# alpc91/SGRL

Measured on AMD Instinct MI355X. Metric: env-steps/sec (whole node) + SET-actor fwd us/step, 3d_walker mix @8192 envs/GPU, higher is better.
Workload: dtype f64 (dynamics) / f32 (SET actor, obs); 1 GPU; 3D_Walker++ 8 variants x 1024 envs per GPU (config 3), random U(-1,1) actions, auto-reset, SET actor forward on every step, random-init weights; envs_per_gpu=8192, obs_max_len=287, action_max_len=21, replay_gather=none (single rank)

## Files before the change

### include/sgrl_set.h

```cpp
#ifndef SGRL_SET_H
#define SGRL_SET_H

#include <stdint.h>

#ifdef __cplusplus
extern "C" {
#endif

typedef struct sgrl_set sgrl_set;

enum {
  SGRL_SET_EMB0 = 0, SGRL_SET_EMB1, SGRL_SET_EMB2, SGRL_SET_REL_W, SGRL_SET_REL_B, SGRL_SET_FNORM_W, SGRL_SET_FNORM_B,
  SGRL_SET_GENC, SGRL_SET_ENC_W, SGRL_SET_ENC_B, SGRL_SET_GGPROJ, SGRL_SET_L1G_W, SGRL_SET_L1G_B, SGRL_SET_L2G_W,
  SGRL_SET_L2G_B, SGRL_SET_L1NG_W, SGRL_SET_L1NG_B, SGRL_SET_L2NG_W, SGRL_SET_L2NG_B, SGRL_SET_DECG, SGRL_SET_L1M_W,
  SGRL_SET_L1M_B, SGRL_SET_L2M_W, SGRL_SET_L2M_B, SGRL_SET_GPROJ,
  SGRL_SET_NGLOBAL
};
enum {
  SGRL_SET_A_GPROJ = 0, SGRL_SET_A_LG1_W, SGRL_SET_A_LG1_B, SGRL_SET_A_LG2_W, SGRL_SET_A_LG2_B, SGRL_SET_QKV_W,
  SGRL_SET_QKV_B, SGRL_SET_VG_W, SGRL_SET_NGOUT_W, SGRL_SET_NGOUT_B, SGRL_SET_GOUT_W, SGRL_SET_F_GPROJ2,
  SGRL_SET_F_GPROJ3, SGRL_SET_F_LG1_W, SGRL_SET_F_LG1_B, SGRL_SET_F_LG2_W, SGRL_SET_F_LG2_B, SGRL_SET_L3_W,
  SGRL_SET_L3_B, SGRL_SET_L4_W, SGRL_SET_L4_B, SGRL_SET_L5_W, SGRL_SET_L1_W, SGRL_SET_L1_B, SGRL_SET_L2_W,
  SGRL_SET_L2_B, SGRL_SET_N1_W, SGRL_SET_N1_B, SGRL_SET_N2_W, SGRL_SET_N2_B, SGRL_SET_A_GD,
  SGRL_SET_NLAYER
};
#define SGRL_SET_LAYERS 3
#define SGRL_SET_NW (SGRL_SET_NGLOBAL + SGRL_SET_LAYERS * SGRL_SET_NLAYER)

int sgrl_set_create(sgrl_set** out);
void sgrl_set_destroy(sgrl_set* s);

int sgrl_set_weights(sgrl_set* s, const float* w, const int64_t* offsets, int n_offsets);

enum { SGRL_PACK_COPY = 0, SGRL_PACK_PADCOL = 1, SGRL_PACK_FOLD = 2, SGRL_PACK_STACK = 3, SGRL_PACK_MATMUL = 4, SGRL_PACK_SUBMAT = 5,
       SGRL_PACK_PERM32 = 6 };
typedef struct sgrl_pack_seg {
  int64_t dst;
  const void* src0;
  const void* src1;
  int32_t n;
  int32_t kind;
  int32_t a, b;
  float scale;
  int32_t lda, ldb;
  int32_t reserved;
} sgrl_pack_seg;
#define SGRL_SET_NSITES 7
#define SGRL_SET_NEXTRA 2
int sgrl_set_bind_params(sgrl_set* s, const sgrl_pack_seg* segs, int n_segs, const int64_t* offsets, int n_offsets,
                         int64_t total_floats);

int sgrl_set_hold_weights(sgrl_set* s, int hold);

int sgrl_set_graph(sgrl_set* s, int n_morph, const int32_t* morph_L, const int32_t* morph_count, const int32_t* trav,
                   const float* rel);
#define SGRL_SET_GRAPH_CACHE 128

int sgrl_set_forward(sgrl_set* s, const float* obs, int obs_ld, float* act, int act_ld, float max_action, void* stream);

int sgrl_set_forward_q(sgrl_set* s, const float* obs, int obs_ld, const float* action, int action_ld, float* q, int q_ld,
                       void* stream);

int sgrl_set_num_nodes(const sgrl_set* s);
int64_t sgrl_set_workspace_bytes(const sgrl_set* s);
int64_t sgrl_set_generation(const sgrl_set* s);
int sgrl_set_time_forward(sgrl_set* s, const float* obs, int obs_ld, float* act, int act_ld, float max_action,
                          int reps, void* stream, float* ms_out);
int sgrl_set_peek(sgrl_set* s, int which, float* host, int64_t n_floats);
int sgrl_set_debug_stop_after(sgrl_set* s, int stage);
int sgrl_set_debug_small_nodes(sgrl_set* s, int nodes);
int sgrl_set_last_split(const sgrl_set* s);
#define SGRL_SET_FORM_F16X3 2
#define SGRL_SET_FORM_BF16X6 3
int sgrl_set_gemm_form(sgrl_set* s, int form);
int sgrl_set_debug_product(sgrl_set* s, int kind, int form, const float* A, int lda, const float* W, int ldw, const float* bias,
                           float* C, int ldc, int M, int N, int K, const float* rowdiv, const float* aux_in, float* aux_out,
                           void* stream);
int sgrl_set_debug_chain(sgrl_set* s, int kind, const float* A, int lda, int K, const float* Wp, const float* W1, const float* b1, int hid,
                         const float* W2, const float* b2, float* C, int ldc, int M, const float* rowdiv, const float* ln, float* zc,
                         float* z2, float* fn, void* stream);
long long sgrl_set_debug_redos(int reset);
const char* sgrl_set_last_error(void);

#ifdef __cplusplus
}
#endif
#endif
```

### sgrl_amd/csrc/set_actor.hip

```cpp
#include <hip/hip_runtime.h>

#include <algorithm>
#include <cmath>
#include <cstdint>
#include <cstdlib>
#include <cstring>
#include <string>
#include <type_traits>
#include <vector>

#include "../../include/sgrl.h"
#include "../../include/sgrl_set.h"
#include "../../include/sgrl_train.h"
#include "gemm_f32.h"
#include "chain_f16.h"
#include "stream_pick.h"

namespace {

thread_local std::string g_set_err;
int sfail(int code, const std::string& msg) { g_set_err = msg; return code; }
#define SHIP_TRY(expr)                                                                     \
  do {                                                                                     \
    hipError_t _e = (expr);                                                                \
    if (_e != hipSuccess) return sfail(SGRL_ERR_HIP, std::string(#expr) + ": " + hipGetErrorString(_e)); \
  } while (0)

constexpr int D = 128;
constexpr int ZD = 32;
constexpr int GK = sgrl_gemm::kGramK;
constexpr int OGLD = 144;

using sgrl_gemm::EPI_ACC2;
using sgrl_gemm::EPI_EQUIV;
using sgrl_gemm::EPI_LN;
using sgrl_gemm::EPI_RELU;
using sgrl_gemm::EPI_ROWDIV;
using sgrl_gemm::EPI_ZSPLIT;
using sgrl_gemm::GemmArgs;
using sgrl_gemm::k_gemm2;

__device__ __forceinline__ float wave_sum_f32(float v) {
  for (int off = 32; off > 0; off >>= 1) v += __shfl_xor(v, off, 64);
  return v;
}

struct NodeTab {
  const int32_t* node_env;
  const int32_t* node_limb;
  const int32_t* node_mnode;
  const int32_t* trav;
  int TM;
};
constexpr int kEmbedNodes = 8;
__global__ __launch_bounds__(128) void k_embed(const float* __restrict__ obs, int obs_ld, const float* __restrict__ action,
                                               int act_ld, int ngf, NodeTab nt, const float* Wge, const float* We,
                                               const float* be, const float* e0, const float* e1, const float* e2, float* g,
                                               float* cat, float* outg, float* outng, float* gdir, float* zc, float* z2, int N) {
  __shared__ float os[kEmbedNodes][44];
  const int n0 = blockIdx.x * kEmbedNodes, c = threadIdx.x;
  for (int idx = c; idx < kEmbedNodes * 44; idx += 128) {
    const int q = idx / 44, k = idx % 44, n = n0 + q;
    float v = 0.f;
    if (n < N) {
      const int env = nt.node_env[n], limb = nt.node_limb[n];
      if (k < 41) v = obs[(size_t)env * obs_ld + 41 * limb + k];
      else if (action) v = action[(size_t)env * act_ld + 3 * limb + (k - 41)];
    }
    os[q][k] = v;
  }
  float wg[8], we[20];
#pragma unroll
  for (int j = 0; j < 8; j++) wg[j] = Wge[c * 8 + j];
#pragma unroll
  for (int j = 0; j < 20; j++) we[j] = j < ngf ? We[c * ngf + j] : 0.f;
  const float bias = be[c];
  __syncthreads();
  const float sc = sqrtf(128.f);
  for (int q = 0; q < kEmbedNodes; q++) {
    const int n = n0 + q;
    if (n >= N) break;
    const float* o = os[q];
    const int mn = nt.node_mnode[n];
    for (int s = 0; s < 3; s++) {
      float v = 0.f;
#pragma unroll
      for (int j = 0; j < 8; j++) v += wg[j] * o[3 * j + s];
      g[((size_t)n * 3 + s) * D + c] = v * sc;
    }
    float v = bias;
#pragma unroll
    for (int j = 0; j < 20; j++) if (j < ngf) v += we[j] * o[24 + j];
    float pos;
    if (c < 42) pos = e0[nt.trav[mn] * 42 + c];
    else if (c < 84) pos = e1[nt.trav[nt.TM + mn] * 42 + (c - 42)];
    else pos = e2[nt.trav[2 * nt.TM + mn] * 44 + (c - 84)];
    cat[(size_t)n * 256 + 128 + c] = v * sc + pos;
    if (c < 24) { const int s = c / 8, j = c % 8; outg[((size_t)n * 3 + s) * OGLD + j] = o[3 * j + s]; }
    if (c < ngf) outng[(size_t)n * 160 + c] = o[24 + c];
    if (c >= ngf && c < 32) outng[(size_t)n * 160 + 128 + c] = 0.f;
    if (c < 6) {
      const int s = c / 2, e = c % 2;
      const float gv = o[3 * (1 + e) + s];
      gdir[((size_t)n * 3 + s) * 2 + e] = gv;
      zc[((size_t)n * 3 + s) * ZD + 30 + e] = gv;
      z2[((size_t)n * 3 + s) * ZD + 30 + e] = gv;
    }
  }
}

__global__ void k_stack_proj(const float* __restrict__ Wp, const float* __restrict__ Wq, int C, int Cpad, float* out) {
  for (int i = blockIdx.x * blockDim.x + threadIdx.x; i < 64 * Cpad; i += gridDim.x * blockDim.x) {
    const int r = i / Cpad, c = i % Cpad;
    float v = 0.f;
    if (c < C) {
      if (r < 30) v = Wp[r * C + c];
      else if (Wq && r >= 32 && r < 62) v = Wq[(r - 32) * C + c];
    }
    out[i] = v;
  }
}

constexpr int PACK_CHUNK = 4096;
constexpr int PACK_CHUNK_MM = 256;
__global__ __launch_bounds__(256) void k_pack(const sgrl_pack_seg* __restrict__ segs, const int2* __restrict__ chunks,
                                              const unsigned short* __restrict__ tri, float* w) {
  const int2 ch = chunks[blockIdx.x];
  const sgrl_pack_seg sg = segs[ch.x];
  const float* s0 = static_cast<const float*>(sg.src0);
  const float* s1 = static_cast<const float*>(sg.src1);
  const int end = min(ch.y + (sg.kind == SGRL_PACK_MATMUL ? PACK_CHUNK_MM : PACK_CHUNK), sg.n);
  for (int i = ch.y + (int)threadIdx.x; i < end; i += 256) {
    float v = 0.f;
    switch (sg.kind) {
      case SGRL_PACK_COPY:
        if (i < sg.a) v = s0[i] * sg.scale;
        break;
      case SGRL_PACK_PADCOL: {
        const int r = i / sg.b, c = i % sg.b;
        if (c < sg.a) v = s0[(size_t)r * sg.a + c];
        break;
      }
      case SGRL_PACK_FOLD: {
        const int r = i / GK, k = i % GK;
        const unsigned short t = tri[k];
        if (t != 0xFFFF) {
          const int aa = t >> 8, bb = t & 255;
          const float* row = s0 + (size_t)r * (ZD * ZD);
          v = (aa == bb) ? row[aa * ZD + bb] : row[aa * ZD + bb] + row[bb * ZD + aa];
        }
        break;
      }
      case SGRL_PACK_STACK: {
        const int r = i / sg.b, c = i % sg.b;
        if (c < sg.a) {
          if (r < 30) v = s0[r * sg.a + c];
          else if (s1 && r >= 32 && r < 62) v = s1[(r - 32) * sg.a + c];
        }
        break;
      }
      case SGRL_PACK_MATMUL: {
        const int r = i / sg.b, c = i % sg.b;
        const float* ar = s0 + (size_t)r * sg.lda;
        float acc = 0.f;
        int k = 0;
        for (; k + 8 <= sg.a; k += 8) {
          float x[8], y[8];
#pragma unroll
          for (int u = 0; u < 8; u++) { x[u] = ar[k + u]; y[u] = s1[(size_t)(k + u) * sg.ldb + c]; }
#pragma unroll
          for (int u = 0; u < 8; u++) acc += x[u] * y[u];
        }
        for (; k < sg.a; k++) acc += ar[k] * s1[(size_t)k * sg.ldb + c];
        v = acc * sg.scale;
        break;
      }
      case SGRL_PACK_PERM32: {
        const int r = i / sg.a, k = i % sg.a;
        v = s0[(size_t)((r & 31) * 32 + (r >> 5)) * sg.a + k];
        break;
      }
      case SGRL_PACK_SUBMAT: {
        const int r = i / sg.b, c = i % sg.b;
        v = s0[(size_t)r * sg.lda + c];
        break;
      }
      default: break;
    }
    w[sg.dst + i] = v;
  }
}

__global__ void k_relbias(const float* rel, const float* Wr, const float* br, float* relb, const int32_t* m_off,
                          const int32_t* m_L, int n_morph) {
  const int k = blockIdx.x;
  if (k >= n_morph) return;
  const int L = m_L[k], off = m_off[k];
  for (int i = threadIdx.x; i < 2 * L * L; i += blockDim.x) {
    const int h = i / (L * L), ij = i % (L * L);
    const float* r = rel + (size_t)(off / 2) * 3 + ij * 3;
    relb[off + i] = Wr[h * 3] * r[0] + Wr[h * 3 + 1] * r[1] + Wr[h * 3 + 2] * r[2] + br[h];
  }
}

struct EnvTab {
  const int32_t* env_off;
  const int32_t* env_L;
  const int32_t* env_relb;
};
__global__ __launch_bounds__(256) void k_attention(const float* __restrict__ qkv, const float* __restrict__ U,
                                                   const float* __restrict__ gdir, const float* relb, EnvTab et,
                                                   int use_bias, const float* __restrict__ b_ng, const float* __restrict__ GD,
                                                   float* delta_dbg, float* g1, float* ng, int ng_ld,
                                                   const float* __restrict__ ln_w, const float* __restrict__ ln_b) {
  constexpr int LMAX = 14;
  __shared__ float sc[2 * LMAX * LMAX];
  __shared__ float gd[2 * LMAX * 3 * 2];
  __shared__ float dl[LMAX][128];
  const int e = blockIdx.x, t = threadIdx.x;
  const int n0 = et.env_off[e], L = et.env_L[e];
  {
    const int sub = t & 7;
    for (int idx = t >> 3; idx < 2 * L * L; idx += 32) {
      const int h = idx / (L * L), i = (idx / L) % L, j = idx % L;
      const float4* q = reinterpret_cast<const float4*>(qkv + (size_t)(n0 + i) * 768 + h * 128);
      const float4* k = reinterpret_cast<const float4*>(qkv + (size_t)(n0 + j) * 768 + 256 + h * 128);
      float s = 0.f;
#pragma unroll
      for (int u = 0; u < 4; u++) {
        const float4 a = q[sub + 8 * u], b = k[sub + 8 * u];
        s += a.x * b.x + a.y * b.y + a.z * b.z + a.w * b.w;
      }
      s += __shfl_xor(s, 1, 64); s += __shfl_xor(s, 2, 64); s += __shfl_xor(s, 4, 64);
      if (sub == 0) sc[idx] = use_bias ? s + relb[et.env_relb[e] + idx] : s;
    }
  }
  __syncthreads();
  if (t < 2 * L) {
    float* row = sc + t * L;
    float mx = row[0];
    for (int j = 1; j < L; j++) mx = fmaxf(mx, row[j]);
    float sum = 0.f;
    for (int j = 0; j < L; j++) { row[j] = expf(row[j] - mx); sum += row[j]; }
    for (int j = 0; j < L; j++) row[j] = row[j] / sum;
  }
  __syncthreads();
  for (int idx = t; idx < 2 * L * 6; idx += 256) {
    const int h = idx / (L * 6), i = (idx / 6) % L, se = idx % 6;
    const float* w = sc + (h * L + i) * L;
    float s = 0.f;
    for (int j = 0; j < L; j++) s += w[j] * gdir[(size_t)(n0 + j) * 6 + se];
    gd[idx] = s;
  }
  __syncthreads();
  {
    const int quantity = t >> 6, ln = t & 63, h = ln >> 5, c4 = (ln & 31) * 4;
    const float* vbase = quantity == 0 ? qkv + (size_t)n0 * 768 + 512 + h * 128 + c4
                                       : U + ((size_t)n0 * 3 + (quantity - 1)) * 256 + h * 128 + c4;
    auto body = [&](auto ltc, const int i0) __attribute__((always_inline)) {
      constexpr int LT = decltype(ltc)::value;
      float4 out[LT];
#pragma unroll
      for (int i = 0; i < LT; i++) out[i] = make_float4(0.f, 0.f, 0.f, 0.f);
      const float* wh = sc + h * L * L;
      if (L <= 8) {
#pragma unroll
        for (int jb = 0; jb < 8; jb += 4) {
          if (jb >= L) break;
          float4 v[4];
#pragma unroll
          for (int j = 0; j < 4; j++)
            v[j] = jb + j < L ? *reinterpret_cast<const float4*>(vbase + (size_t)(jb + j) * 768) : make_float4(0.f, 0.f, 0.f, 0.f);
#pragma unroll
          for (int j = 0; j < 4; j++)
            if (jb + j < L) {
#pragma unroll
              for (int i = 0; i < LT; i++)
                if (i0 + i < L) {
                  const float w = wh[(i0 + i) * L + jb + j];
                  out[i].x += w * v[j].x; out[i].y += w * v[j].y; out[i].z += w * v[j].z; out[i].w += w * v[j].w;
                }
            }
        }
      } else {
        float4 v = *reinterpret_cast<const float4*>(vbase);
        for (int j = 0; j < L; j++) {
          const float4 vn = *reinterpret_cast<const float4*>(vbase + (size_t)(j + 1 < L ? j + 1 : j) * 768);
#pragma unroll
          for (int i = 0; i < LT; i++)
            if (i0 + i < L) {
              const float w = wh[(i0 + i) * L + j];
              out[i].x += w * v.x; out[i].y += w * v.y; out[i].z += w * v.z; out[i].w += w * v.w;
            }
          v = vn;
        }
      }
      if (quantity != 0) {
        const float4 ga = *reinterpret_cast<const float4*>(GD + (h * 128 + c4) * 2);
        const float4 gb = *reinterpret_cast<const float4*>(GD + (h * 128 + c4) * 2 + 4);
#pragma unroll
        for (int i = 0; i < LT; i++)
          if (i0 + i < L) {
            const float* gg = gd + (h * L + i0 + i) * 6 + 2 * (quantity - 1);
            const float g0 = gg[0], g1v = gg[1];
            out[i].x += ga.x * g0 + ga.y * g1v; out[i].y += ga.z * g0 + ga.w * g1v;
            out[i].z += gb.x * g0 + gb.y * g1v; out[i].w += gb.z * g0 + gb.w * g1v;
          }
      }
      float4 bb = make_float4(0.f, 0.f, 0.f, 0.f);
      if (quantity == 0) bb = *reinterpret_cast<const float4*>(b_ng + c4);
#pragma unroll
      for (int i = 0; i < LT; i++)
        if (i0 + i < L) {
          float4 o = out[i];
          const float px = __shfl_xor(o.x, 32, 64), py = __shfl_xor(o.y, 32, 64), pz = __shfl_xor(o.z, 32, 64), pw = __shfl_xor(o.w, 32, 64);
          o = h == 0 ? make_float4(o.x + px, o.y + py, o.z + pz, o.w + pw) : make_float4(px + o.x, py + o.y, pz + o.z, pw + o.w);
          if ((i & 1) == h) {
            if (quantity != 0) {
              *reinterpret_cast<float4*>(g1 + ((size_t)(n0 + i0 + i) * 3 + (quantity - 1)) * 128 + c4) = o;
            } else {
              o.x += bb.x; o.y += bb.y; o.z += bb.z; o.w += bb.w;
              *reinterpret_cast<float4*>(&dl[i0 + i][c4]) = o;
              if (delta_dbg) *reinterpret_cast<float4*>(delta_dbg + (size_t)(n0 + i0 + i) * 128 + c4) = o;
            }
          }
        }
    };
    for (int i0 = 0; i0 < L; i0 += 4) body(std::integral_constant<int, 4>{}, i0);
  }
  __syncthreads();
  const int lane = t & 63;
  const float w0 = ln_w[lane], w1 = ln_w[64 + lane], b0 = ln_b[lane], b1 = ln_b[64 + lane];
  for (int i = t >> 6; i < L; i += 4) {
    float* row = ng + (size_t)(n0 + i) * ng_ld;
    const float v0 = row[lane] + dl[i][lane], v1 = row[64 + lane] + dl[i][64 + lane];
    const float mu = wave_sum_f32(v0 + v1) * (1.f / 128.f);
    const float d0 = v0 - mu, d1 = v1 - mu;
    const float var = wave_sum_f32(d0 * d0 + d1 * d1) * (1.f / 128.f);
    const float inv = 1.0f / sqrtf(var + 1e-5f);
    row[lane] = d0 * inv * w0 + b0;
    row[64 + lane] = d1 * inv * w1 + b1;
  }
}

__global__ __launch_bounds__(256) void k_add_ln(const float* x, int ldx, const float* delta, int ldd, const float* w,
                                                const float* b, float* out1, int ld1, float* out2, int ld2, int N) {
  const int row = blockIdx.x * 4 + (threadIdx.x >> 6), lane = threadIdx.x & 63;
  if (row >= N) return;
  float v0 = x[(size_t)row * ldx + lane], v1 = x[(size_t)row * ldx + 64 + lane];
  if (delta) { v0 += delta[(size_t)row * ldd + lane]; v1 += delta[(size_t)row * ldd + 64 + lane]; }
  const float mu = wave_sum_f32(v0 + v1) * (1.f / 128.f);
  const float d0 = v0 - mu, d1 = v1 - mu;
  const float var = wave_sum_f32(d0 * d0 + d1 * d1) * (1.f / 128.f);
  const float inv = 1.0f / sqrtf(var + 1e-5f);
  const float y0 = d0 * inv * w[lane] + b[lane], y1 = d1 * inv * w[64 + lane] + b[64 + lane];
  if (out1) { out1[(size_t)row * ld1 + lane] = y0; out1[(size_t)row * ld1 + 64 + lane] = y1; }
  if (out2) { out2[(size_t)row * ld2 + lane] = y0; out2[(size_t)row * ld2 + 64 + lane] = y1; }
}

__global__ __launch_bounds__(128) void k_equiv(const float* __restrict__ T, const float* __restrict__ W5,
                                               const float* __restrict__ g1, float* g, float* outg, int N) {
  __shared__ float Ts[8 * 96];
  const int t = threadIdx.x, n0 = blockIdx.x * 8;
  const int rows = min(8, N - n0) * 3;
  for (int o = t; o < 8 * 96; o += 128) Ts[o] = (n0 + o / 96 < N) ? T[(size_t)n0 * 96 + o] : 0.f;
  float w[32];
#pragma unroll
  for (int c = 0; c < 32; c++) w[c] = W5[t * 32 + c];
  __syncthreads();
#pragma unroll
  for (int rb = 0; rb < 24; rb += 8) {
    if (rb >= rows) break;
    float gv[8], g1v[8];
#pragma unroll
    for (int r = 0; r < 8; r++) {
      const size_t row = (size_t)n0 * 3 + (rb + r < rows ? rb + r : 0);
      gv[r] = g[row * D + t];
      g1v[r] = g1[row * D + t];
    }
#pragma unroll
    for (int r = 0; r < 8; r++) {
      if (rb + r >= rows) break;
      const float* tt = Ts + (rb + r) * 32;
      float v = 0.f;
#pragma unroll
      for (int c = 0; c < 32; c++) v += tt[c] * w[c];
      const size_t row = (size_t)n0 * 3 + rb + r;
      const float gn = gv[r] + (g1v[r] + v);
      g[row * D + t] = gn;
      if (outg) {
        outg[row * OGLD + 8 + t] = gn;
        if (t < OGLD - 136) outg[row * OGLD + 136 + t] = 0.f;
      }
    }
  }
}

__global__ __launch_bounds__(128) void k_head_out(const float* __restrict__ T, const float* __restrict__ wdec,
                                                  const float* __restrict__ obs, int obs_ld, NodeTab nt, float* act, int act_ld,
                                                  float max_action, int N) {
  const int n = blockIdx.x * 4 + (threadIdx.x >> 5), c = threadIdx.x & 31;
  if (n >= N) return;
  float vec[3];
  const float wd = wdec[c];
  for (int s = 0; s < 3; s++) {
    float v = T[(size_t)n * 96 + s * 32 + c] * wd;
    for (int off = 16; off > 0; off >>= 1) v += __shfl_xor(v, off, 32);
    vec[s] = v;
  }
  if (c < 3) {
    const int env = nt.node_env[n], limb = nt.node_limb[n];
    const float* o = obs + (size_t)env * obs_ld + 41 * limb + 3 * (5 + c);
    const float a = o[0] * vec[0] + o[1] * vec[1] + o[2] * vec[2];
    act[(size_t)env * act_ld + 3 * limb + c] = max_action * tanhf(a);
  }
}


__global__ __launch_bounds__(128) void k_head_out2(const float* __restrict__ m2, const float* __restrict__ z, const float* __restrict__ obs,
                                                   int obs_ld, NodeTab nt, float* act, int act_ld, float max_action, int N) {
  const int n = blockIdx.x * 4 + (threadIdx.x >> 5), c = threadIdx.x & 31;
  if (n >= N) return;
  float vec[3];
  const float mq = m2[(size_t)n * 32 + c];
  for (int s = 0; s < 3; s++) {
    float v = z[(size_t)n * 96 + s * 32 + c] * mq;
    for (int off = 16; off > 0; off >>= 1) v += __shfl_xor(v, off, 32);
    vec[s] = v;
  }
  if (c < 3) {
    const int env = nt.node_env[n], limb = nt.node_limb[n];
    const float* o = obs + (size_t)env * obs_ld + 41 * limb + 3 * (5 + c);
    const float a = o[0] * vec[0] + o[1] * vec[1] + o[2] * vec[2];
    act[(size_t)env * act_ld + 3 * limb + c] = max_action * tanhf(a);
  }
}

__global__ __launch_bounds__(256) void k_q_head(const float* __restrict__ c, const float* __restrict__ w, const float* __restrict__ b,
                                                const float* __restrict__ fn, NodeTab nt, float* q, int q_ld, int N) {
  const int n = blockIdx.x * 4 + (threadIdx.x >> 6), lane = threadIdx.x & 63;
  if (n >= N) return;
  const float* row = c + (size_t)n * 256;
  float v = row[lane] * w[lane] + row[64 + lane] * w[64 + lane] + row[128 + lane] * w[128 + lane] + row[192 + lane] * w[192 + lane];
  v = wave_sum_f32(v);
  if (lane == 0) q[(size_t)nt.node_env[n] * q_ld + nt.node_limb[n]] = (v + b[0]) / fn[n];
}

}

struct GraphCfg {
  std::vector<int32_t> key_i;
  std::vector<float> key_f;
  int n_env = 0, N = 0, n_morph = 0, TM = 0, Lmax = 0;
  int split_env = 0, split_node = 0;
  int32_t *d_node_env = nullptr, *d_node_limb = nullptr, *d_node_mnode = nullptr, *d_trav = nullptr;
  int32_t *d_env_off = nullptr, *d_env_L = nullptr, *d_env_relb = nullptr, *d_m_off = nullptr, *d_m_L = nullptr;
  float *d_rel = nullptr, *d_relb = nullptr;
  uint64_t last_use = 0;
  void release() {
    void* ptrs[] = {d_node_env, d_node_limb, d_node_mnode, d_trav, d_env_off, d_env_L, d_env_relb, d_m_off, d_m_L, d_rel, d_relb};
    for (void* q : ptrs) if (q) (void)hipFree(q);
  }
};

struct sgrl_set {
  const float* w = nullptr;
  int64_t off[SGRL_SET_NW];
  bool have_w = false, have_graph = false;
  int n_env = 0, N = 0, n_morph = 0, TM = 0, Lmax = 0;
  int split_env = 0, split_node = 0;
  int last_split = 0;
  int32_t *d_node_env = nullptr, *d_node_limb = nullptr, *d_node_mnode = nullptr, *d_trav = nullptr;
  int32_t *d_env_off = nullptr, *d_env_L = nullptr, *d_env_relb = nullptr, *d_m_off = nullptr, *d_m_L = nullptr;
  float *d_rel = nullptr, *d_relb = nullptr;
  std::vector<GraphCfg*> cfgs;
  uint64_t use_clock = 0;
  int64_t generation = 0;
  float* ws = nullptr;
  int64_t ws_floats = 0;
  int carved_N = 0;
  float* cat_cur = nullptr;
  float *g, *cat, *cat2, *zc, *fn, *h256, *qkv, *vg, *g1, *z2, *mat, *t256, *t256b, *t128a, *t128b, *delta,
      *outg, *outng, *gdir;
  float* wstack = nullptr;
  const float* site_ptr[SGRL_SET_NSITES];
  bool hold = false, packed_ok = false;
  int packed_form = 0;
  hipEvent_t ev_pack = nullptr;
  const float* l2mf_w = nullptr;
  const float* l2mf_b = nullptr;
  unsigned short* d_tri = nullptr;
  bool stack_dirty = true;
  bool stack_critic = false;
  int stop_after = -1;
  int small_nodes = -1;
  int gemm_form = 0;
  sgrl_gemm::EncMat* d_enc = nullptr;
  int n_enc = 0, enc_rows = 0;
  float* wsc = nullptr;
  std::vector<std::pair<int64_t, int>> enc_index;
  bool live = false;
  float* wflat = nullptr;
  unsigned* wwords = nullptr;
  int64_t wflat_floats = 0;
  sgrl_pack_seg* d_segs = nullptr;
  int2* d_chunks = nullptr;
  int n_chunks = 0;
  hipStream_t side = nullptr;
  hipEvent_t ev_fork = nullptr, ev_join = nullptr, ev_l3 = nullptr;
  hipEvent_t ev_fork_b = nullptr, ev_join_b = nullptr, ev_split = nullptr, ev_merge = nullptr;
  std::vector<hipStream_t> side_ok_for;
  int side_picks = 0;
  const float* W(int slot) const { return w + off[slot]; }
  const float* WL(int layer, int k) const { return w + off[SGRL_SET_NGLOBAL + layer * SGRL_SET_NLAYER + k]; }
};

namespace {

constexpr int64_t kPerNodeFloats = 384  + 256 + 256  + 96  + 1  + 256  + 768  +
                                   768  + 384  + 96  + 96  + 256 + 256  +
                                   128 + 128 + 128  + 3 * OGLD  + 160  + 6 ;
constexpr int kWsArrays = 19;

int64_t ws_floats_for(int64_t N) { return kPerNodeFloats * N + 32 * kWsArrays; }

void free_graphs(sgrl_set* s) {
  for (GraphCfg* c : s->cfgs) { c->release(); delete c; }
  s->cfgs.clear();
  if (s->ws) (void)hipFree(s->ws);
  s->ws = nullptr; s->ws_floats = 0; s->carved_N = 0;
  s->have_graph = false;
}

template <class T>
int upload(T** dst, const std::vector<T>& v) {
  if (hipMalloc(dst, sizeof(T) * (v.size() ? v.size() : 1)) != hipSuccess) return -1;
  if (!v.empty() && hipMemcpy(*dst, v.data(), sizeof(T) * v.size(), hipMemcpyHostToDevice) != hipSuccess) return -1;
  return 0;
}

void pick_split(const std::vector<int32_t>& env_off, int N, int* env_out, int* node_out) {
  int best = 0, best_rank = -1;
  int64_t best_dist = 0;
  for (size_t e = 1; e < env_off.size(); e++) {
    const int n = env_off[e];
    const int64_t dist = std::abs(2 * (int64_t)n - N);
    const int rank = 2 * dist > N / 16 ? 0 : (n % 128 == 0 ? 3 : n % 64 == 0 ? 2 : 1);
    if (best_rank < 0 || rank > best_rank || (rank == best_rank && dist < best_dist)) { best = (int)e; best_rank = rank; best_dist = dist; }
  }
  *env_out = best;
  *node_out = best ? env_off[best] : 0;
}

int use_cfg(sgrl_set* s, GraphCfg* c) {
  const int64_t N = c->N;
  const int64_t need = ws_floats_for(N);
  if (need > s->ws_floats) {
    if (s->ws) { (void)hipFree(s->ws); s->generation++; }
    s->ws = nullptr; s->ws_floats = 0; s->carved_N = 0;
    if (hipMalloc(&s->ws, sizeof(float) * need) != hipSuccess) return sfail(SGRL_ERR_HIP, "device allocation failed (SET workspace)");
    s->ws_floats = need;
  }
  if (s->carved_N != c->N) {
    float* p = s->ws;
    auto take = [&](int64_t n) { float* r = p; p += (n + 31) & ~int64_t(31); return r; };
    s->g = take(384 * N); s->cat = take(256 * N); s->cat2 = take(256 * N); s->zc = take(96 * N); s->fn = take(N);
    s->h256 = take(256 * N); s->qkv = take(768 * N); s->vg = take(768 * N);
    s->g1 = take(384 * N); s->z2 = take(96 * N); s->mat = take(96 * N); s->t256 = take(256 * N); s->t256b = take(256 * N); s->t128a = take(128 * N);
    s->t128b = take(128 * N); s->delta = take(128 * N); s->outg = take(3 * OGLD * N); s->outng = take(160 * N); s->gdir = take(6 * N);
    if (p - s->ws > s->ws_floats) return sfail(SGRL_ERR_LIMIT, "workspace carve-up overflow");
    s->carved_N = c->N;
  }
  s->n_env = c->n_env; s->N = c->N; s->n_morph = c->n_morph; s->TM = c->TM; s->Lmax = c->Lmax;
  s->split_env = c->split_env; s->split_node = c->split_node;
  s->d_node_env = c->d_node_env; s->d_node_limb = c->d_node_limb; s->d_node_mnode = c->d_node_mnode; s->d_trav = c->d_trav;
  s->d_env_off = c->d_env_off; s->d_env_L = c->d_env_L; s->d_env_relb = c->d_env_relb; s->d_m_off = c->d_m_off; s->d_m_L = c->d_m_L;
  s->d_rel = c->d_rel; s->d_relb = c->d_relb;
  c->last_use = ++s->use_clock;
  s->have_graph = true;
  return SGRL_OK;
}

bool gemm_use_split() {
  static const bool v = [] { const char* e = getenv("SGRL_SET_GEMM"); return !(e && e[0] == 'f'); }();
  return v;
}
struct GemmCtx {
  int form = SGRL_SET_FORM_F16X3;
  const float* w_base = nullptr; const unsigned* w_words = nullptr;
  const float* wsc = nullptr;
  const std::vector<std::pair<int64_t, int>>* enc_index = nullptr;
};
int gemm_default_form() {
  static const int v = [] { const char* e = getenv("SGRL_SET_GEMM"); return (e && e[0] == 'b') ? SGRL_SET_FORM_BF16X6 : SGRL_SET_FORM_F16X3; }();
  return v;
}
const float* wsc_of(const GemmCtx& gx, const float* W) {
  if (!gx.enc_index) return nullptr;
  const int64_t off = W - gx.w_base;
  for (const auto& e : *gx.enc_index) if (e.first == off) return gx.wsc + e.second;
  return nullptr;
}
GemmArgs with_words(const GemmCtx& gx, const GemmArgs& a) {
  GemmArgs b = a;
  b.W = reinterpret_cast<const float*>(gx.w_words + (a.W - gx.w_base));
  b.wscale = wsc_of(gx, a.W);
  return b;
}
template <int F> struct GemmKernels {
  static constexpr auto kNarrow = k_gemm2<F, 4, 1, 1, 2, 16, 1>;
  static constexpr auto kWide = k_gemm2<F, 4, 2, 1, 2, 32, 2>;
  static constexpr auto kSquare = k_gemm2<F, 4, 4, 1, 1, 32, 2>;
  static constexpr auto kSplit = sgrl_gemm::k_gemm3<F, 4, 2, 1, 2, 16, 2>;
  static constexpr auto kSplitH = sgrl_gemm::k_gemm3<F, 4, 2, 1, 2, 16, 2, false, false, false, 0, false, 2, true, 2>;
  static constexpr int kSplitHLds = sgrl_gemm::TileCfg3<4, 2, 1, 2, 16, 2>::kLdsBytes;
  static constexpr int kNarrowLds = sgrl_gemm::TileCfg<4, 1, 1, 2, 16>::kLdsBytes;
  static constexpr int kWideLds = sgrl_gemm::TileCfg<4, 2, 1, 2, 32>::kLdsBytes;
  static constexpr int kSquareLds = sgrl_gemm::TileCfg<4, 4, 1, 1, 32>::kLdsBytes;
  static constexpr int kSplitLds = sgrl_gemm::TileCfg3<4, 2, 1, 2, 16>::kLdsBytes;
  static bool raise_lds_limits() {
    return hipFuncSetAttribute(reinterpret_cast<const void*>(kNarrow), hipFuncAttributeMaxDynamicSharedMemorySize, kNarrowLds) == hipSuccess &&
           hipFuncSetAttribute(reinterpret_cast<const void*>(kWide), hipFuncAttributeMaxDynamicSharedMemorySize, kWideLds) == hipSuccess &&
           hipFuncSetAttribute(reinterpret_cast<const void*>(kSquare), hipFuncAttributeMaxDynamicSharedMemorySize, kSquareLds) == hipSuccess &&
           hipFuncSetAttribute(reinterpret_cast<const void*>(kSplit), hipFuncAttributeMaxDynamicSharedMemorySize, kSplitLds) == hipSuccess &&
           hipFuncSetAttribute(reinterpret_cast<const void*>(kSplitH), hipFuncAttributeMaxDynamicSharedMemorySize, kSplitHLds) == hipSuccess;
  }
  static void launch(const GemmCtx& gx, hipStream_t st, const GemmArgs& a) {
    const int tiles128 = ((a.M + 127) / 128) * ((a.N + 127) / 128);
    if (a.N <= 64 || (a.K % 32) != 0) {
      hipLaunchKernelGGL(kNarrow, dim3(((a.M + 127) / 128) * ((a.N + 63) / 64)), dim3(256), kNarrowLds, st, a);
    } else if (gemm_use_split()) {
      if (gx.form == SGRL_SET_FORM_F16X3) hipLaunchKernelGGL(kSplitH, dim3(tiles128), dim3(512), kSplitHLds, st, with_words(gx, a));
      else hipLaunchKernelGGL(kSplit, dim3(tiles128), dim3(512), kSplitLds, st, a);
    } else if (tiles128 < 512) {
      hipLaunchKernelGGL(kNarrow, dim3(((a.M + 127) / 128) * ((a.N + 63) / 64)), dim3(256), kNarrowLds, st, a);
    } else if (a.N >= 512) {
      hipLaunchKernelGGL(kWide, dim3(tiles128), dim3(512), kWideLds, st, a);
    } else {
      hipLaunchKernelGGL(kSquare, dim3(tiles128), dim3(1024), kSquareLds, st, a);
    }
  }
};

constexpr auto kProjH = sgrl_gemm::k_gemm3<EPI_ZSPLIT, 4, 1, 1, 2, 16, 2, false, false, false, 0, false, 2, false, 2>;
constexpr int kProjHLds = sgrl_gemm::TileCfg3<4, 1, 1, 2, 16, 2>::kLdsBytes;

constexpr auto kGemmEquiv = sgrl_gemm::k_gemm3<EPI_ROWDIV | EPI_EQUIV, 4, 2, 1, 2, 16, 2>;
constexpr auto kGemmEquivH = sgrl_gemm::k_gemm3<EPI_ROWDIV | EPI_EQUIV, 4, 2, 1, 2, 16, 2, false, false, false, 0, false, 2, true, 2>;
constexpr int kEquivLds = GemmKernels<0>::kSplitLds > 128 * 100 * 4 ? GemmKernels<0>::kSplitLds : 128 * 100 * 4;
int launch_gemm_equiv(const GemmCtx& gx, hipStream_t st, const float* A, int lda, const float* W, int ldw, const float* bias, int M, int K,
                      const float* rowdiv, const float* zq, float* tout) {
  if (K % 32 != 0 || (lda & 3) || (ldw & 3)) return sfail(SGRL_ERR_ARG, "gemm_equiv: K must be a multiple of 32 and rows 16-byte aligned");
  GemmArgs a{A, lda, W, ldw, bias, nullptr, 0, M, 1024, K, EPI_ROWDIV | EPI_EQUIV, rowdiv, nullptr, 0};
  a.zq = zq; a.tout = tout;
  if (gx.form == SGRL_SET_FORM_F16X3) hipLaunchKernelGGL(kGemmEquivH, dim3(((M + 127) / 128) * 8), dim3(512), kEquivLds, st, with_words(gx, a));
  else hipLaunchKernelGGL(kGemmEquiv, dim3(((M + 127) / 128) * 8), dim3(512), kEquivLds, st, a);
  return SGRL_OK;
}

constexpr auto kGemmGram = sgrl_gemm::k_gemm3<EPI_RELU, 4, 2, 1, 2, 16, 2, false, false, false, 0, true>;
constexpr auto kGemmGramH = sgrl_gemm::k_gemm3<EPI_RELU, 4, 2, 1, 2, 16, 2, false, false, false, 0, true, 2, true, 2>;
int launch_gemm_gram(const GemmCtx& gx, hipStream_t st, const float* zc, const float* W, const float* bias, float* C, int ldc, int M, int N, float* fn) {
  if (N % 128 != 0) return sfail(SGRL_ERR_ARG, "gemm_gram: N must be a multiple of 128");
  GemmArgs a{zc, 96, W, GK, bias, C, ldc, M, N, GK, EPI_RELU, nullptr, nullptr, 0};
  a.rowdiv_out = fn;
  if (gx.form == SGRL_SET_FORM_F16X3) hipLaunchKernelGGL(kGemmGramH, dim3(((M + 127) / 128) * (N / 128)), dim3(512), GemmKernels<0>::kSplitHLds, st, with_words(gx, a));
  else hipLaunchKernelGGL(kGemmGram, dim3(((M + 127) / 128) * (N / 128)), dim3(512), GemmKernels<0>::kSplitLds, st, a);
  return SGRL_OK;
}

constexpr auto kGemmLn = sgrl_gemm::k_gemm3<EPI_ROWDIV | EPI_LN, 4, 2, 1, 2, 16, 2>;
constexpr auto kGemmLnH = sgrl_gemm::k_gemm3<EPI_ROWDIV | EPI_LN, 4, 2, 1, 2, 16, 2, false, false, false, 0, false, 2, true, 2>;
int launch_gemm_ln(const GemmCtx& gx, hipStream_t st, const float* A, int lda, const float* W, int ldw, const float* bias, int M, int K,
                   const float* rowdiv, float* ln_io, int ln_ld, const float* ln_w, const float* ln_b) {
  if (K % 32 != 0 || (lda & 3) || (ldw & 3)) return sfail(SGRL_ERR_ARG, "gemm_ln: K must be a multiple of 32 and rows 16-byte aligned");
  GemmArgs a{A, lda, W, ldw, bias, nullptr, 0, M, 128, K, EPI_ROWDIV | EPI_LN, rowdiv, nullptr, 0};
  a.ln_io = ln_io; a.ln_ld = ln_ld; a.ln_w = ln_w; a.ln_b = ln_b;
  if (gx.form == SGRL_SET_FORM_F16X3) hipLaunchKernelGGL(kGemmLnH, dim3((M + 127) / 128), dim3(512), GemmKernels<0>::kSplitHLds, st, with_words(gx, a));
  else hipLaunchKernelGGL(kGemmLn, dim3((M + 127) / 128), dim3(512), GemmKernels<0>::kSplitLds, st, a);
  return SGRL_OK;
}

int launch_gemm(const GemmCtx& gx, hipStream_t st, const float* A, int lda, const float* W, int ldw, const float* bias, float* C, int ldc,
                int M, int N, int K, int flags = 0, const float* rowdiv = nullptr, float* C2 = nullptr, int ldc2 = 0) {
  if (K % 16 != 0 || (lda & 3) || (ldw & 3)) return sfail(SGRL_ERR_ARG, "gemm: K must be a multiple of 16 and rows 16-byte aligned");
  GemmArgs a{A, lda, W, ldw, bias, C, ldc, M, N, K, flags, rowdiv, C2, ldc2};
  switch (flags) {
    case 0: GemmKernels<0>::launch(gx, st, a); break;
    case EPI_RELU: GemmKernels<EPI_RELU>::launch(gx, st, a); break;
    case EPI_ROWDIV: GemmKernels<EPI_ROWDIV>::launch(gx, st, a); break;
    case EPI_ACC2: GemmKernels<EPI_ACC2>::launch(gx, st, a); break;
    default: return sfail(SGRL_ERR_ARG, "gemm: unsupported epilogue combination");
  }
  return SGRL_OK;
}

bool chain_enabled() {
  static const bool v = [] { const char* e = getenv("SGRL_SET_CHAIN"); return !(e && e[0] == '0'); }();
  return v;
}
using sgrl_gemm::ChainArgs;
using sgrl_gemm::k_chain;
constexpr auto kSiteA = k_chain<1, 256, 0, 1>;
constexpr auto kSiteF = k_chain<1, 256, 0, 2>;
constexpr auto kSiteH1 = k_chain<1, 128, 0, 1>;
constexpr auto kSiteH2 = k_chain<1, 128, 0, 2>;
constexpr auto kChainLn = k_chain<0, 256, EPI_ROWDIV | EPI_LN, 0>;
constexpr auto kChainNg = k_chain<0, 128, 0, 0>;
constexpr auto kChainPlain = k_chain<0, 256, 0, 0>;
bool chain_raise_lds_limits() {
  const void* ks[] = {reinterpret_cast<const void*>(kSiteA), reinterpret_cast<const void*>(kSiteF), reinterpret_cast<const void*>(kSiteH1),
                      reinterpret_cast<const void*>(kSiteH2), reinterpret_cast<const void*>(kChainLn), reinterpret_cast<const void*>(kChainNg),
                      reinterpret_cast<const void*>(kChainPlain)};
  for (const void* k : ks)
    if (hipFuncSetAttribute(k, hipFuncAttributeMaxDynamicSharedMemorySize, sgrl_gemm::kChainLds) != hipSuccess) return false;
  return hipFuncSetAttribute(reinterpret_cast<const void*>(k_chain<0, 256, EPI_ROWDIV | EPI_EQUIV, 0>), hipFuncAttributeMaxDynamicSharedMemorySize,
                             sgrl_gemm::kChainEqLds) == hipSuccess;
}
const unsigned* words_of(const GemmCtx& gx, const float* W) { return gx.w_words + (W - gx.w_base); }
int launch_site(const GemmCtx& gx, hipStream_t st, const float* X, int ldx, int Kp, const float* Wp, float* zc, float* z2, float* fn, const float* W1,
                const float* b1, int hid, const float* W2, const float* b2, float* C, int ldc, int M) {
  if (Kp % 16 != 0 || (ldx & 3) || (hid != 256 && hid != 128)) return sfail(SGRL_ERR_ARG, "site: K must be a multiple of 16, rows 16-byte aligned, hidden width 128 or 256");
  ChainArgs a{};
  a.A = zc; a.W1 = words_of(gx, W1); a.ldw1 = GK; a.b1 = b1; a.W2 = words_of(gx, W2); a.ldw2 = hid; a.b2 = b2; a.C = C; a.ldc = ldc; a.M = M; a.K1 = GK;
  a.fn_out = fn; a.X = X; a.ldx = ldx; a.Kp = Kp; a.Wp = words_of(gx, Wp); a.zc = zc; a.z2 = z2;
  a.ws1 = wsc_of(gx, W1); a.ws2 = wsc_of(gx, W2); a.wsp = wsc_of(gx, Wp);
  if (!a.ws1 || !a.ws2 || !a.wsp) return sfail(SGRL_ERR_ARG, "site: a weight operand is not a matrix of the row-scale table");
  const dim3 grid((M + sgrl_gemm::kChainRows - 1) / sgrl_gemm::kChainRows);
  if (hid == 256) {
    if (z2) hipLaunchKernelGGL(kSiteF, grid, dim3(512), sgrl_gemm::kChainLds, st, a);
    else hipLaunchKernelGGL(kSiteA, grid, dim3(512), sgrl_gemm::kChainLds, st, a);
  } else {
    if (z2) hipLaunchKernelGGL(kSiteH2, grid, dim3(512), sgrl_gemm::kChainLds, st, a);
    else hipLaunchKernelGGL(kSiteH1, grid, dim3(512), sgrl_gemm::kChainLds, st, a);
  }
  return SGRL_OK;
}
int launch_chain_ln(const GemmCtx& gx, hipStream_t st, const float* A, int lda, int K1, const float* W1, const float* b1, const float* W2, const float* b2,
                    const float* rowdiv, float* ln_io, int ln_ld, const float* ln_w, const float* ln_b, int M, float* ln_out = nullptr) {
  if (K1 % 16 != 0 || (lda & 3)) return sfail(SGRL_ERR_ARG, "chain: K must be a multiple of 16 and rows 16-byte aligned");
  ChainArgs a{};
  a.A = A; a.lda = lda; a.W1 = words_of(gx, W1); a.ldw1 = K1; a.b1 = b1; a.W2 = words_of(gx, W2); a.ldw2 = 256; a.b2 = b2; a.M = M; a.K1 = K1;
  a.rowdiv = rowdiv; a.ln_io = ln_io; a.ln_ld = ln_ld; a.ln_w = ln_w; a.ln_b = ln_b; a.ln_out = ln_out;
  a.ws1 = wsc_of(gx, W1); a.ws2 = wsc_of(gx, W2);
  if (!a.ws1 || !a.ws2) return sfail(SGRL_ERR_ARG, "chain: a weight operand is not a matrix of the row-scale table");
  hipLaunchKernelGGL(kChainLn, dim3((M + sgrl_gemm::kChainRows - 1) / sgrl_gemm::kChainRows), dim3(512), sgrl_gemm::kChainLds, st, a);
  return SGRL_OK;
}
constexpr auto kChainEq = k_chain<0, 256, EPI_ROWDIV | EPI_EQUIV, 0>;
int launch_chain_ng(const GemmCtx& gx, hipStream_t st, const float* A, int lda, int K1, const float* W1, const float* b1, const float* W2, const float* b2,
                    float* C, int ldc, int M) {
  if (K1 % 16 != 0 || (lda & 3)) return sfail(SGRL_ERR_ARG, "chain: K must be a multiple of 16 and rows 16-byte aligned");
  ChainArgs a{};
  a.A = A; a.lda = lda; a.W1 = words_of(gx, W1); a.ldw1 = K1; a.b1 = b1; a.W2 = words_of(gx, W2); a.ldw2 = 128; a.b2 = b2; a.C = C; a.ldc = ldc; a.M = M;
  a.K1 = K1; a.ws1 = wsc_of(gx, W1); a.ws2 = wsc_of(gx, W2);
  if (!a.ws1 || !a.ws2) return sfail(SGRL_ERR_ARG, "chain: a weight operand is not a matrix of the row-scale table");
  hipLaunchKernelGGL(kChainNg, dim3((M + sgrl_gemm::kChainRows - 1) / sgrl_gemm::kChainRows), dim3(512), sgrl_gemm::kChainLds, st, a);
  return SGRL_OK;
}

constexpr int kSmallNodesDefault = 2048;
constexpr int kSplitMinNodes = 2048;

__global__ __launch_bounds__(256) void k_gram576(const float* __restrict__ zc, const unsigned short* __restrict__ tri,
                                                 float* __restrict__ A, float* __restrict__ fn, int N) {
  __shared__ float zs[4][96];
  const int w = threadIdx.x >> 6, lane = threadIdx.x & 63, node = blockIdx.x * 4 + w;
  const bool live = node < N;
  if (live) {
    zs[w][lane] = zc[(size_t)node * 96 + lane];
    if (lane < 32) zs[w][64 + lane] = zc[(size_t)node * 96 + 64 + lane];
  }
  __syncthreads();
  if (!live) return;
  float ss = 0.f;
  for (int k = lane; k < GK; k += 64) {
    const unsigned t = tri[k];
    float v = 0.f;
    if (t != 0xFFFFu) {
      const int a = t >> 8, b = t & 255;
      v = zs[w][a] * zs[w][b] + zs[w][32 + a] * zs[w][32 + b] + zs[w][64 + a] * zs[w][64 + b];
      ss += (a == b ? 1.f : 2.f) * v * v;
    }
    A[(size_t)node * GK + k] = v;
  }
  ss = wave_sum_f32(ss);
  if (lane == 0) fn[node] = sqrtf(ss) + 1.f;
}

__global__ __launch_bounds__(128) void k_zmat_perm(const float* __restrict__ zq, const float* __restrict__ matp,
                                                   float* __restrict__ tout) {
  __shared__ float ms[32 * 33], zs[96];
  const int t = threadIdx.x;
  const size_t n = blockIdx.x;
  for (int o = t; o < 1024; o += 128) ms[(o >> 5) * 33 + (o & 31)] = matp[n * 1024 + o];
  if (t < 96) zs[t] = zq[n * 96 + t];
  __syncthreads();
  if (t >= 96) return;
  const int sI = t >> 5, c = t & 31;
  float acc = 0.f;
#pragma unroll
  for (int a = 0; a < 32; a++) acc += zs[sI * 32 + a] * ms[c * 33 + a];
  tout[n * 96 + t] = acc;
}

int small_fail() { return sfail(SGRL_ERR_HIP, std::string("small-batch product: ") + sgrl_train_last_error()); }

int small_gemm(hipStream_t st, const float* A, int lda, const float* W, int ldw, const float* bias, float* C, int ldc, int M,
               int N, int K, int flags = 0, const float* rowdiv = nullptr) {
  if (flags & ~(EPI_RELU | EPI_ROWDIV)) return sfail(SGRL_ERR_ARG, "small gemm: unsupported epilogue");
  const int rc = sgrl_linear_forward(A, lda, W, ldw, bias, (flags & EPI_ROWDIV) ? rowdiv : nullptr, C, ldc, M, N, K,
                                     (flags & EPI_RELU) ? 1 : 0, st);
  return rc == SGRL_OK ? rc : small_fail();
}

struct Part {
  int r0, M, e0, ne;
  hipStream_t st, sd;
  hipEvent_t ev_fork, ev_join;
  hipEvent_t ev_site0;
  float *catc, *cato, *g, *zc, *z2, *fn, *h256, *qkv, *vg, *g1, *mat, *t256, *t256b, *t128a, *t128b, *delta, *outg, *outng;
  NodeTab nt;
};

constexpr int kStages = 4 * SGRL_SET_LAYERS + 2, kStop = 1;

struct Forward {
  sgrl_set* s;
  const float* obs; int obs_ld; float* act; int act_ld; float max_action;
  bool critic; const float* action; int action_ld;
  hipStream_t st, sd;
  bool capturing, one_stream;
  bool small, chain;
  int ngf;
  GemmCtx gx;
  NodeTab nt;
  EnvTab et;

  void fork(const Part& p) const { if (!one_stream && p.sd != p.st) { (void)hipEventRecord(p.ev_fork, p.st); (void)hipStreamWaitEvent(p.sd, p.ev_fork, 0); } }
  void join(const Part& p) const { if (!one_stream && p.sd != p.st) { (void)hipEventRecord(p.ev_join, p.sd); (void)hipStreamWaitEvent(p.st, p.ev_join, 0); } }

  Part part(int r0, int M, int e0, int ne, hipStream_t pst, hipStream_t psd, hipEvent_t ev_fork, hipEvent_t ev_join, hipEvent_t ev_site0) const {
    const size_t r = (size_t)r0;
    Part p{r0, M, e0, ne, pst, psd, ev_fork, ev_join, ev_site0};
    p.catc = s->cat + 256 * r; p.cato = s->cat2 + 256 * r; p.g = s->g + 384 * r; p.zc = s->zc + 96 * r; p.z2 = s->z2 + 96 * r; p.fn = s->fn + r;
    p.h256 = s->h256 + 256 * r; p.qkv = s->qkv + 768 * r; p.vg = s->vg + 768 * r; p.g1 = s->g1 + 384 * r; p.mat = s->mat + 96 * r;
    p.t256 = s->t256 + 256 * r; p.t256b = s->t256b + 256 * r; p.t128a = s->t128a + 128 * r; p.t128b = s->t128b + 128 * r;
    p.delta = s->delta + 128 * r; p.outg = s->outg + 3 * OGLD * r; p.outng = s->outng + 160 * r;
    p.nt = NodeTab{nt.node_env + r, nt.node_limb + r, nt.node_mnode + r, nt.trav, nt.TM};
    return p;
  }
  const float* site_w(int site) const { return s->live ? s->site_ptr[site] : s->wstack + (size_t)site * 64 * 128; }

  int gemm(hipStream_t q, const float* A, int lda, const float* W, int ldw, const float* bias, float* C, int ldc, int M, int N, int K,
           int flags = 0, const float* rowdiv = nullptr) const {
    return small ? small_gemm(q, A, lda, W, ldw, bias, C, ldc, M, N, K, flags, rowdiv) : launch_gemm(gx, q, A, lda, W, ldw, bias, C, ldc, M, N, K, flags, rowdiv);
  }
  int gram_gemm(const Part& p, const float* W, const float* b, float* C, int ldc, int Nout) const {
    if (!small) return launch_gemm_gram(gx, p.st, p.zc, W, b, C, ldc, p.M, Nout, p.fn);
    hipLaunchKernelGGL(k_gram576, dim3((p.M + 3) / 4), dim3(256), 0, p.st, p.zc, s->d_tri, p.qkv, p.fn, p.M);
    return small_gemm(p.st, p.qkv, GK, W, GK, b, C, ldc, p.M, Nout, GK, EPI_RELU);
  }
  int equiv_gemm(const Part& p, const float* A, const float* W, const float* b) const {
    if (!small) return launch_gemm_equiv(gx, p.st, A, 256, W, 256, b, p.M, 256, p.fn, p.z2, p.mat);
    const int rc = small_gemm(p.st, A, 256, W, 256, b, p.qkv, 1024, p.M, 1024, 256, EPI_ROWDIV, p.fn);
    if (rc != SGRL_OK) return rc;
    hipLaunchKernelGGL(k_zmat_perm, dim3(p.M), dim3(128), 0, p.st, p.z2, p.qkv, p.mat);
    return SGRL_OK;
  }
  int project(const Part& p, const float* X, int ldx, int K, int site, float* z2) const {
    if (K % 16 != 0 || (ldx & 3)) return sfail(SGRL_ERR_ARG, "projection: K must be a multiple of 16 and rows 16-byte aligned");
    if (small) {
      int rc = small_gemm(p.st, X, ldx, site_w(site), K, nullptr, p.zc, ZD, 3 * p.M, 30, K);
      if (rc == SGRL_OK && z2) rc = small_gemm(p.st, X, ldx, site_w(site) + (size_t)32 * K, K, nullptr, z2, ZD, 3 * p.M, 30, K);
      return rc;
    }
    GemmArgs a{X, ldx, site_w(site), K, nullptr, p.zc, ZD, 3 * p.M, z2 ? 64 : 32, K, EPI_ZSPLIT, nullptr, z2, ZD};
    if (gx.form == SGRL_SET_FORM_F16X3 && gemm_use_split())
      hipLaunchKernelGGL(kProjH, dim3(((a.M + 127) / 128) * ((a.N + 63) / 64)), dim3(256), kProjHLds, p.st, with_words(gx, a));
    else
      GemmKernels<EPI_ZSPLIT>::launch(gx, p.st, a);
    return SGRL_OK;
  }
  int site(const Part& p, const float* X, int ldx, int K, int site, float* z2, const float* W1, const float* b1, int hid, float* hbuf,
           const float* W2, const float* b2, float* C) const {
    if (chain) return launch_site(gx, p.st, X, ldx, K, site_w(site), p.zc, z2, p.fn, W1, b1, hid, W2, b2, C, 256, p.M);
    int rc = project(p, X, ldx, K, site, z2);
    if (rc == SGRL_OK) rc = gram_gemm(p, W1, b1, hbuf, hid, hid);
    if (rc == SGRL_OK) rc = gemm(p.st, hbuf, hid, W2, hid, b2, C, 256, p.M, 128, hid);
    return rc;
  }

  void prologue(const Part& whole) {
    const int N = s->N;
    (void)hipMemsetAsync(act, 0, sizeof(float) * (size_t)s->n_env * act_ld, st);
    const bool want_words = !small && gx.form == SGRL_SET_FORM_F16X3 && gemm_use_split();
    const bool reuse = s->live && s->hold && s->packed_ok && (!want_words || s->packed_form == SGRL_SET_FORM_F16X3) && !capturing;
    if (reuse) (void)hipStreamWaitEvent(st, s->ev_pack, 0);
    if (s->live && !reuse)
      hipLaunchKernelGGL(k_pack, dim3(s->n_chunks), dim3(256), 0, st, s->d_segs, s->d_chunks, s->d_tri, s->wflat);
    const bool encode = s->live && !reuse && want_words;
    if (encode) {
      fork(whole);
      hipLaunchKernelGGL(sgrl_gemm::k_encode_rows, dim3((s->enc_rows + 3) / 4), dim3(256), 0, sd, s->wflat, s->wwords, s->wsc, s->d_enc, s->n_enc,
                         s->enc_rows);
    }
    hipLaunchKernelGGL(k_relbias, dim3(s->n_morph), dim3(256), 0, st, s->d_rel, s->W(SGRL_SET_REL_W), s->W(SGRL_SET_REL_B),
                       s->d_relb, s->d_m_off, s->d_m_L, s->n_morph);
    hipLaunchKernelGGL(k_embed, dim3((N + kEmbedNodes - 1) / kEmbedNodes), dim3(128), 0, st, obs, obs_ld, action, action_ld, ngf, nt,
                       s->W(SGRL_SET_GENC), s->W(SGRL_SET_ENC_W), s->W(SGRL_SET_ENC_B), s->W(SGRL_SET_EMB0), s->W(SGRL_SET_EMB1),
                       s->W(SGRL_SET_EMB2), s->g, s->cat, s->outg, s->outng, s->gdir, s->zc, s->z2, N);
    if (encode) join(whole);
    if (s->live && !reuse && !capturing) {
      s->packed_ok = s->hold;
      s->packed_form = want_words ? SGRL_SET_FORM_F16X3 : SGRL_SET_FORM_BF16X6;
      if (s->hold) (void)hipEventRecord(s->ev_pack, st);
    }
    s->cat_cur = s->cat;
    if (!s->live && (s->stack_dirty || s->stack_critic != critic)) {
      s->stack_critic = critic;
      auto sw = [&](int site) { return s->wstack + (size_t)site * 64 * 128; };
      for (int l = 0; l < SGRL_SET_LAYERS; l++) {
        hipLaunchKernelGGL(k_stack_proj, dim3(32), dim3(256), 0, st, s->WL(l, SGRL_SET_A_GPROJ), (const float*)nullptr, D, D, sw(2 * l));
        hipLaunchKernelGGL(k_stack_proj, dim3(32), dim3(256), 0, st, s->WL(l, SGRL_SET_F_GPROJ2), s->WL(l, SGRL_SET_F_GPROJ3), D, D, sw(2 * l + 1));
      }
      hipLaunchKernelGGL(k_stack_proj, dim3(36), dim3(256), 0, st, s->W(SGRL_SET_GGPROJ), critic ? (const float*)nullptr : s->W(SGRL_SET_GPROJ), 136, OGLD, sw(6));
      s->stack_dirty = false;
    }
  }
  int attn_site(const Part& p, int l) const {
    fork(p);
    int rc = gemm(p.sd, p.g, D, s->WL(l, SGRL_SET_VG_W), D, nullptr, p.vg, 256, 3 * p.M, 256, D);
    if (rc == SGRL_OK)
      rc = site(p, p.g, D, D, 2 * l, nullptr, s->WL(l, SGRL_SET_A_LG1_W), s->WL(l, SGRL_SET_A_LG1_B), 256, p.h256, s->WL(l, SGRL_SET_A_LG2_W),
                s->WL(l, SGRL_SET_A_LG2_B), p.catc);
    if (rc != SGRL_OK) return rc;
    if (l == 0 && p.ev_site0) (void)hipEventRecord(p.ev_site0, p.st);
    rc = gemm(p.st, p.catc, 256, s->WL(l, SGRL_SET_QKV_W), 256, s->WL(l, SGRL_SET_QKV_B), p.qkv, 768, p.M, 768, 256, EPI_ROWDIV, p.fn);
    if (rc != SGRL_OK) return rc;
    join(p);
    return SGRL_OK;
  }
  int attention(const Part& p, int l) const {
    const EnvTab etp{et.env_off + p.e0, et.env_L + p.e0, et.env_relb + p.e0};
    hipLaunchKernelGGL(k_attention, dim3(p.ne), dim3(256), 0, p.st, s->qkv, s->vg, s->gdir, s->d_relb, etp, l == 0 ? 1 : 0,
                       s->WL(l, SGRL_SET_NGOUT_B), s->WL(l, SGRL_SET_A_GD), s->stop_after == 2 * l ? s->delta : (float*)nullptr,
                       s->g1, p.catc - 256 * (size_t)p.r0 + 128, 256, s->WL(l, SGRL_SET_N1_W), s->WL(l, SGRL_SET_N1_B));
    return s->stop_after == 2 * l ? kStop : SGRL_OK;
  }
  int ffn_site(const Part& p, int l) const {
    return site(p, p.g1, D, D, 2 * l + 1, p.z2, s->WL(l, SGRL_SET_F_LG1_W), s->WL(l, SGRL_SET_F_LG1_B), 256, p.h256, s->WL(l, SGRL_SET_F_LG2_W),
                s->WL(l, SGRL_SET_F_LG2_B), p.catc);
  }
  int norm2_unfused(const Part& p, int l) const {
    float* const ng = p.catc + 128;
    if (!one_stream) {
      (void)hipEventRecord(s->ev_l3, p.st);
      (void)hipStreamWaitEvent(p.sd, s->ev_l3, 0);
    }
    if (!small)
      return launch_gemm_ln(gx, p.sd, p.t256b, 256, s->WL(l, SGRL_SET_L2_W), 256, s->WL(l, SGRL_SET_L2_B), p.M, 256, p.fn, ng, 256,
                            s->WL(l, SGRL_SET_N2_W), s->WL(l, SGRL_SET_N2_B));
    const int rc = small_gemm(p.st, p.t256b, 256, s->WL(l, SGRL_SET_L2_W), 256, s->WL(l, SGRL_SET_L2_B), p.delta, 128, p.M, 128, 256, EPI_ROWDIV, p.fn);
    if (rc != SGRL_OK) return rc;
    hipLaunchKernelGGL(k_add_ln, dim3((p.M + 3) / 4), dim3(256), 0, p.st, ng, 256, p.delta, 128, s->WL(l, SGRL_SET_N2_W),
                       s->WL(l, SGRL_SET_N2_B), (float*)nullptr, 0, ng, 256, p.M);
    return SGRL_OK;
  }
  int ffn_tail(Part& p, int l) const {
    fork(p);
    int rc;
    if (chain) {
      rc = launch_chain_ln(gx, p.sd, p.catc, 256, 256, s->WL(l, SGRL_SET_L1_W), s->WL(l, SGRL_SET_L1_B), s->WL(l, SGRL_SET_L2_W), s->WL(l, SGRL_SET_L2_B),
                           p.fn, p.catc + 128, 256, s->WL(l, SGRL_SET_N2_W), s->WL(l, SGRL_SET_N2_B), p.M, p.cato + 128);
    } else {
      rc = gemm(p.sd, p.catc, 256, s->WL(l, SGRL_SET_L1_W), 256, s->WL(l, SGRL_SET_L1_B), p.t256b, 256, p.M, 256, 256, EPI_RELU);
    }
    if (rc == SGRL_OK) rc = gemm(p.st, p.catc, 256, s->WL(l, SGRL_SET_L3_W), 256, s->WL(l, SGRL_SET_L3_B), p.t256, 256, p.M, 256, 256, EPI_RELU);
    if (rc == SGRL_OK && !chain) rc = norm2_unfused(p, l);
    if (rc == SGRL_OK) rc = equiv_gemm(p, p.t256, s->WL(l, SGRL_SET_L4_W), s->WL(l, SGRL_SET_L4_B));
    if (rc != SGRL_OK) return rc;
    hipLaunchKernelGGL(k_equiv, dim3((p.M + 7) / 8), dim3(128), 0, p.st, p.mat, s->WL(l, SGRL_SET_L5_W), p.g1, p.g,
                       l == SGRL_SET_LAYERS - 1 ? p.outg : (float*)nullptr, p.M);
    join(p);
    if (chain) {
      std::swap(p.catc, p.cato);
      s->cat_cur = p.catc - 256 * (size_t)p.r0;
    }
    return s->stop_after == 2 * l + 1 ? kStop : SGRL_OK;
  }
  int head_site(const Part& p) const {
    hipLaunchKernelGGL(k_add_ln, dim3((p.M + 3) / 4), dim3(256), 0, p.st, p.catc + 128, 256, (const float*)nullptr, 0, s->W(SGRL_SET_FNORM_W),
                       s->W(SGRL_SET_FNORM_B), (float*)nullptr, 0, p.outng + ngf, 160, p.M);
    fork(p);
    int rc;
    if (chain) {
      rc = launch_chain_ng(gx, p.sd, p.outng, 160, 160, s->W(SGRL_SET_L1NG_W), s->W(SGRL_SET_L1NG_B), s->W(SGRL_SET_L2NG_W), s->W(SGRL_SET_L2NG_B),
                           p.cato + 128, 256, p.M);
    } else {
      rc = gemm(p.sd, p.outng, 160, s->W(SGRL_SET_L1NG_W), 160, s->W(SGRL_SET_L1NG_B), p.t128b, D, p.M, D, 160, EPI_RELU);
      if (rc == SGRL_OK) rc = gemm(p.sd, p.t128b, D, s->W(SGRL_SET_L2NG_W), D, s->W(SGRL_SET_L2NG_B), p.cato + 128, 256, p.M, D, D);
    }
    if (rc == SGRL_OK)
      rc = site(p, p.outg, OGLD, OGLD, 6, critic ? (float*)nullptr : p.z2, s->W(SGRL_SET_L1G_W), s->W(SGRL_SET_L1G_B), 128, p.t128a,
                s->W(SGRL_SET_L2G_W), s->W(SGRL_SET_L2G_B), p.cato);
    if (rc != SGRL_OK) return rc;
    join(p);
    return SGRL_OK;
  }
  int head_out(const Part& p) const {
    const int N = p.M;
    if (critic) {
      hipLaunchKernelGGL(k_q_head, dim3((N + 3) / 4), dim3(256), 0, p.st, p.cato, s->W(SGRL_SET_DECG), s->W(SGRL_SET_L1M_B), p.fn, p.nt, act, act_ld, N);
      return SGRL_OK;
    }
    int rc = gemm(p.st, p.cato, 256, s->W(SGRL_SET_L1M_W), 256, s->W(SGRL_SET_L1M_B), p.t256, 256, N, 256, 256, EPI_RELU);
    if (rc != SGRL_OK) return rc;
    if (!small && s->live && s->l2mf_w) {
      rc = gemm(p.st, p.t256, 256, s->l2mf_w, 256, s->l2mf_b, p.mat, 32, N, 32, 256, EPI_ROWDIV, p.fn);
      if (rc != SGRL_OK) return rc;
      hipLaunchKernelGGL(k_head_out2, dim3((N + 3) / 4), dim3(128), 0, p.st, p.mat, p.z2, obs, obs_ld, p.nt, act, act_ld, max_action, N);
      return SGRL_OK;
    }
    rc = equiv_gemm(p, p.t256, s->W(SGRL_SET_L2M_W), s->W(SGRL_SET_L2M_B));
    if (rc != SGRL_OK) return rc;
    hipLaunchKernelGGL(k_head_out, dim3((N + 3) / 4), dim3(128), 0, p.st, p.mat, s->W(SGRL_SET_DECG), obs, obs_ld, p.nt, act, act_ld, max_action, N);
    return SGRL_OK;
  }
  int stage(Part& p, int k) const {
    const int l = k / 4;
    if (k == 4 * SGRL_SET_LAYERS) return head_site(p);
    if (k > 4 * SGRL_SET_LAYERS) return head_out(p);
    switch (k % 4) {
      case 0: return attn_site(p, l);
      case 1: return attention(p, l);
      case 2: return ffn_site(p, l);
      default: return ffn_tail(p, l);
    }
  }
};

GemmCtx gemm_ctx_of(const sgrl_set* s) {
  GemmCtx gx;
  gx.form = s->gemm_form ? s->gemm_form : gemm_default_form();
  if (!s->live || !s->wwords) gx.form = SGRL_SET_FORM_BF16X6;
  if (!gemm_use_split()) gx.form = SGRL_SET_FORM_BF16X6;
  gx.w_base = s->w; gx.w_words = s->wwords; gx.wsc = s->wsc; gx.enc_index = &s->enc_index;
  return gx;
}

int run_forward(sgrl_set* s, const float* obs, int obs_ld, float* act, int act_ld, float max_action, hipStream_t st,
                bool critic = false, const float* action = nullptr, int action_ld = 0) {
  const int N = s->N;
  Forward f{s, obs, obs_ld, act, act_ld, max_action, critic, action, action_ld, st};
  f.gx = gemm_ctx_of(s);
  f.ngf = critic ? 20 : 17;
  f.nt = NodeTab{s->d_node_env, s->d_node_limb, s->d_node_mnode, s->d_trav, s->TM};
  f.et = EnvTab{s->d_env_off, s->d_env_L, s->d_env_relb};
  f.small = N <= (s->small_nodes >= 0 ? s->small_nodes : kSmallNodesDefault);
  f.chain = !f.small && chain_enabled() && gemm_use_split() && f.gx.form == SGRL_SET_FORM_F16X3;
  hipStreamCaptureStatus cap = hipStreamCaptureStatusNone;
  (void)hipStreamIsCapturing(st, &cap);
  static const bool serial_env = [] { const char* e = getenv("SGRL_SET_ONE_STREAM"); return e && e[0] == '1'; }();
  f.capturing = cap != hipStreamCaptureStatusNone;
  f.one_stream = f.small || f.capturing || serial_env;
  if (!f.one_stream && sgrl_streams::enabled() && s->side_picks < 6 &&
      std::find(s->side_ok_for.begin(), s->side_ok_for.end(), st) == s->side_ok_for.end()) {
    s->side_picks++;
    hipStream_t chosen = sgrl_streams::pick({st}, s->side);
    if (chosen != s->side) s->side_ok_for.clear();
    s->side = chosen;
    s->side_ok_for.push_back(st);
  }
  hipStream_t sd = f.sd = f.one_stream ? st : s->side;
  Part whole = f.part(0, N, 0, s->n_env, st, sd, s->ev_fork, s->ev_join, nullptr);
  f.prologue(whole);
  static const int split_mode = [] { const char* e = getenv("SGRL_SET_SPLIT"); return e && e[0] >= '0' && e[0] <= '3' ? e[0] - '0' : 1; }();
  const bool split = split_mode != 0 && f.chain && !f.one_stream && s->stop_after < 0 && N >= kSplitMinNodes && s->split_node > 0 && s->split_node < N;
  s->last_split = split ? s->split_node : 0;
  if (!split) {
    for (int k = 0; k < kStages; k++) {
      const int rc = f.stage(whole, k);
      if (rc == kStop) return SGRL_OK;
      if (rc != SGRL_OK) return rc;
    }
  } else {
    const bool head_start = split_mode == 3;
    Part a = f.part(0, s->split_node, 0, s->split_env, st, sd, s->ev_fork, s->ev_join, head_start ? s->ev_split : (hipEvent_t) nullptr);
    Part b = f.part(s->split_node, N - s->split_node, s->split_env, s->n_env - s->split_env, sd, st, s->ev_fork_b, s->ev_join_b, nullptr);
    if (split_mode == 1) { a.sd = a.st; b.sd = b.st; }
    if (!head_start) (void)hipEventRecord(s->ev_split, st);
    for (int k = 0; k <= kStages; k++) {
      int rc = k < kStages ? f.stage(a, k) : SGRL_OK;
      if (rc != SGRL_OK) return rc;
      if (k == 0) (void)hipStreamWaitEvent(sd, s->ev_split, 0);
      if (k > 0) rc = f.stage(b, k - 1);
      if (rc != SGRL_OK) return rc;
    }
    (void)hipEventRecord(s->ev_merge, sd);
    (void)hipStreamWaitEvent(st, s->ev_merge, 0);
  }
  const hipError_t le = hipGetLastError();
  if (le != hipSuccess)
    return sfail(SGRL_ERR_HIP, std::string("kernel launch failed in sgrl_set_forward (") + hipGetErrorName(le) + ": " + hipGetErrorString(le) + ")");
  return SGRL_OK;
}

}

extern "C" {

int sgrl_set_create(sgrl_set** out) {
  if (!out) return sfail(SGRL_ERR_ARG, "out is null");
  int ndev = 0;
  if (hipGetDeviceCount(&ndev) != hipSuccess || ndev == 0) {
    *out = nullptr;
    return sfail(SGRL_ERR_HIP, "no HIP device visible: the SET actor fast path needs an MI355X (there is no CPU fallback)");
  }
  const bool attr_ok = hipFuncSetAttribute(reinterpret_cast<const void*>(kGemmEquiv), hipFuncAttributeMaxDynamicSharedMemorySize, kEquivLds) == hipSuccess &&
                       hipFuncSetAttribute(reinterpret_cast<const void*>(kGemmGram), hipFuncAttributeMaxDynamicSharedMemorySize, GemmKernels<0>::kSplitLds) == hipSuccess &&
                       hipFuncSetAttribute(reinterpret_cast<const void*>(kGemmLn), hipFuncAttributeMaxDynamicSharedMemorySize, GemmKernels<0>::kSplitLds) == hipSuccess &&
                       hipFuncSetAttribute(reinterpret_cast<const void*>(kGemmEquivH), hipFuncAttributeMaxDynamicSharedMemorySize, kEquivLds) == hipSuccess &&
                       hipFuncSetAttribute(reinterpret_cast<const void*>(kGemmGramH), hipFuncAttributeMaxDynamicSharedMemorySize, GemmKernels<0>::kSplitHLds) == hipSuccess &&
                       hipFuncSetAttribute(reinterpret_cast<const void*>(kGemmLnH), hipFuncAttributeMaxDynamicSharedMemorySize, GemmKernels<0>::kSplitHLds) == hipSuccess &&
                       GemmKernels<0>::raise_lds_limits() && GemmKernels<EPI_RELU>::raise_lds_limits() &&
                       GemmKernels<EPI_ROWDIV>::raise_lds_limits() && GemmKernels<EPI_ACC2>::raise_lds_limits() &&
                       GemmKernels<EPI_ZSPLIT>::raise_lds_limits() && chain_raise_lds_limits();
  if (!attr_ok) {
    *out = nullptr;
    return sfail(SGRL_ERR_HIP, "cannot raise the dynamic LDS limit of the GEMM kernel");
  }
  sgrl_set* s = new sgrl_set();
  std::vector<unsigned short> tri(GK, (unsigned short)0xFFFF);
  for (int A = 0, o = 0; A < ZD / 4; A++)
    for (int B = 0; B <= A; B++)
      for (int i = 0; i < 4; i++)
        for (int j = 0; j < 4; j++, o++)
          if (4 * A + i >= 4 * B + j) tri[o] = (unsigned short)(((4 * A + i) << 8) | (4 * B + j));
  const size_t wstack_floats = 6 * 64 * 128 + 64 * OGLD;
  if (hipStreamCreateWithFlags(&s->side, hipStreamNonBlocking) != hipSuccess ||
      hipEventCreateWithFlags(&s->ev_fork, hipEventDisableTiming) != hipSuccess ||
      hipEventCreateWithFlags(&s->ev_join, hipEventDisableTiming) != hipSuccess ||
      hipEventCreateWithFlags(&s->ev_l3, hipEventDisableTiming) != hipSuccess ||
      hipEventCreateWithFlags(&s->ev_fork_b, hipEventDisableTiming) != hipSuccess ||
      hipEventCreateWithFlags(&s->ev_join_b, hipEventDisableTiming) != hipSuccess ||
      hipEventCreateWithFlags(&s->ev_split, hipEventDisableTiming) != hipSuccess ||
      hipEventCreateWithFlags(&s->ev_merge, hipEventDisableTiming) != hipSuccess ||
      hipEventCreateWithFlags(&s->ev_pack, hipEventDisableTiming) != hipSuccess) {
    delete s;
    *out = nullptr;
    return sfail(SGRL_ERR_HIP, "cannot create the side stream of the SET actor");
  }
  if (hipMalloc(&s->wstack, sizeof(float) * wstack_floats) != hipSuccess || hipMalloc(&s->d_tri, sizeof(unsigned short) * GK) != hipSuccess ||
      hipMemcpy(s->d_tri, tri.data(), sizeof(unsigned short) * GK, hipMemcpyHostToDevice) != hipSuccess) {
    if (s->wstack) (void)hipFree(s->wstack);
    if (s->d_tri) (void)hipFree(s->d_tri);
    delete s;
    *out = nullptr;
    return sfail(SGRL_ERR_HIP, "device allocation failed in sgrl_set_create");
  }
  *out = s;
  return SGRL_OK;
}

void sgrl_set_destroy(sgrl_set* s) {
  if (!s) return;
  if (s->side) (void)hipStreamSynchronize(s->side);
  free_graphs(s);
  if (s->wstack) (void)hipFree(s->wstack);
  if (s->d_tri) (void)hipFree(s->d_tri);
  if (s->d_enc) (void)hipFree(s->d_enc);
  if (s->wsc) (void)hipFree(s->wsc);
  if (s->wflat) (void)hipFree(s->wflat);
  if (s->wwords) (void)hipFree(s->wwords);
  if (s->d_segs) (void)hipFree(s->d_segs);
  if (s->d_chunks) (void)hipFree(s->d_chunks);
  if (s->side) (void)hipStreamDestroy(s->side);
  if (s->ev_fork) (void)hipEventDestroy(s->ev_fork);
  if (s->ev_join) (void)hipEventDestroy(s->ev_join);
  if (s->ev_l3) (void)hipEventDestroy(s->ev_l3);
  for (hipEvent_t e : {s->ev_fork_b, s->ev_join_b, s->ev_split, s->ev_merge}) if (e) (void)hipEventDestroy(e);
  if (s->ev_pack) (void)hipEventDestroy(s->ev_pack);
  delete s;
}

int sgrl_set_weights(sgrl_set* s, const float* w, const int64_t* offsets, int n_offsets) {
  if (!s || !w || !offsets || n_offsets != SGRL_SET_NW) return sfail(SGRL_ERR_ARG, "sgrl_set_weights: bad argument");
  s->w = w;
  std::memcpy(s->off, offsets, sizeof(int64_t) * SGRL_SET_NW);
  s->have_w = true;
  s->live = false;
  s->l2mf_w = nullptr; s->l2mf_b = nullptr;
  s->stack_dirty = true;
  return SGRL_OK;
}

int sgrl_set_bind_params(sgrl_set* s, const sgrl_pack_seg* segs, int n_segs, const int64_t* offsets, int n_offsets,
                         int64_t total_floats) {
  if (!s || !segs || n_segs <= 0 || !offsets || n_offsets != SGRL_SET_NW + SGRL_SET_NSITES + SGRL_SET_NEXTRA || total_floats <= 0)
    return sfail(SGRL_ERR_ARG, "sgrl_set_bind_params: bad argument");
  std::vector<int> order(n_segs);
  for (int i = 0; i < n_segs; i++) order[i] = i;
  std::sort(order.begin(), order.end(), [&](int x, int y) { return segs[x].dst < segs[y].dst; });
  int64_t pos = 0;
  std::vector<int2> chunks;
  for (int oi = 0; oi < n_segs; oi++) {
    const sgrl_pack_seg& g = segs[order[oi]];
    if (g.dst != pos || g.n <= 0 || !g.src0) return sfail(SGRL_ERR_ARG, "sgrl_set_bind_params: segments must tile the buffer without gaps");
    bool ok = false;
    switch (g.kind) {
      case SGRL_PACK_COPY: ok = g.a >= 0 && g.a <= g.n; break;
      case SGRL_PACK_PADCOL: ok = g.a > 0 && g.b >= g.a && g.n % g.b == 0; break;
      case SGRL_PACK_FOLD: ok = g.n % GK == 0; break;
      case SGRL_PACK_STACK: ok = g.a > 0 && g.b >= g.a && g.n == 64 * g.b; break;
      case SGRL_PACK_MATMUL: ok = g.src1 && g.a > 0 && g.b > 0 && g.n % g.b == 0 && g.lda >= g.a && g.ldb >= g.b; break;
      case SGRL_PACK_SUBMAT: ok = g.b > 0 && g.n % g.b == 0 && g.lda >= g.b; break;
      case SGRL_PACK_PERM32: ok = g.a > 0 && g.n == 1024 * g.a; break;
      default: break;
    }
    if (!ok) return sfail(SGRL_ERR_ARG, "sgrl_set_bind_params: inconsistent segment " + std::to_string(order[oi]));
    for (int st = 0; st < g.n; st += (g.kind == SGRL_PACK_MATMUL ? PACK_CHUNK_MM : PACK_CHUNK)) chunks.push_back(make_int2(order[oi], st));
    pos += g.n;
  }
  if (pos != total_floats) return sfail(SGRL_ERR_ARG, "sgrl_set_bind_params: segments do not add up to total_floats");
  for (int k = 0; k < n_offsets; k++)
    if (offsets[k] < 0 || offsets[k] >= total_floats || (offsets[k] & 3)) return sfail(SGRL_ERR_ARG, "sgrl_set_bind_params: bad offset");
  if (s->wflat) s->generation++;
  if (s->wflat) (void)hipFree(s->wflat);
  if (s->wwords) (void)hipFree(s->wwords);
  if (s->d_segs) (void)hipFree(s->d_segs);
  if (s->d_chunks) (void)hipFree(s->d_chunks);
  s->wwords = nullptr;
  s->packed_ok = false;
  s->wflat = nullptr; s->d_segs = nullptr; s->d_chunks = nullptr; s->live = false; s->have_w = false;
  if (hipMalloc(&s->wflat, sizeof(float) * total_floats) != hipSuccess ||
      hipMalloc(&s->wwords, sizeof(unsigned) * total_floats) != hipSuccess ||
      hipMalloc(&s->d_segs, sizeof(sgrl_pack_seg) * n_segs) != hipSuccess ||
      hipMalloc(&s->d_chunks, sizeof(int2) * chunks.size()) != hipSuccess ||
      hipMemcpy(s->d_segs, segs, sizeof(sgrl_pack_seg) * n_segs, hipMemcpyHostToDevice) != hipSuccess ||
      hipMemcpy(s->d_chunks, chunks.data(), sizeof(int2) * chunks.size(), hipMemcpyHostToDevice) != hipSuccess)
    return sfail(SGRL_ERR_HIP, "device allocation failed in sgrl_set_bind_params");
  s->wflat_floats = total_floats;
  std::vector<int64_t> bounds(offsets, offsets + n_offsets);
  bounds.push_back(total_floats);
  std::sort(bounds.begin(), bounds.end());
  auto room = [&](int64_t off) { return *std::upper_bound(bounds.begin(), bounds.end(), off) - off; };
  {
    std::vector<sgrl_gemm::EncMat> mats;
    s->enc_index.clear();
    int rows_total = 0;
    auto add = [&](int64_t off, int rows, int K, int group = 1) {
      if (room(off) < (int64_t)rows * K) return;
      mats.push_back(sgrl_gemm::EncMat{off, rows, K, rows_total, group});
      s->enc_index.emplace_back(off, rows_total);
      rows_total += rows;
    };
    add(offsets[SGRL_SET_L1G_W], 128, GK); add(offsets[SGRL_SET_L2G_W], 128, 128);
    add(offsets[SGRL_SET_L1NG_W], 128, 160); add(offsets[SGRL_SET_L2NG_W], 128, 128);
    add(offsets[SGRL_SET_L1M_W], 256, 256); add(offsets[SGRL_SET_L2M_W], 1024, 256, 32);
    for (int l = 0; l < SGRL_SET_LAYERS; l++) {
      const int64_t* o = offsets + SGRL_SET_NGLOBAL + l * SGRL_SET_NLAYER;
      add(o[SGRL_SET_A_LG1_W], 256, GK); add(o[SGRL_SET_A_LG2_W], 128, 256); add(o[SGRL_SET_QKV_W], 768, 256); add(o[SGRL_SET_VG_W], 256, 128);
      add(o[SGRL_SET_F_LG1_W], 256, GK); add(o[SGRL_SET_F_LG2_W], 128, 256); add(o[SGRL_SET_L3_W], 256, 256); add(o[SGRL_SET_L4_W], 1024, 256, 32);
      add(o[SGRL_SET_L1_W], 256, 256); add(o[SGRL_SET_L2_W], 128, 256); add(o[SGRL_SET_L5_W], 128, 32);
    }
    for (int k = 0; k < SGRL_SET_NSITES; k++) add(offsets[SGRL_SET_NW + k], 64, k == 6 ? OGLD : 128);
    if (s->d_enc) (void)hipFree(s->d_enc);
    if (s->wsc) (void)hipFree(s->wsc);
    s->d_enc = nullptr; s->wsc = nullptr;
    s->n_enc = (int)mats.size(); s->enc_rows = rows_total;
    if (hipMalloc(&s->d_enc, sizeof(sgrl_gemm::EncMat) * mats.size()) != hipSuccess || hipMalloc(&s->wsc, sizeof(float) * rows_total) != hipSuccess ||
        hipMemcpy(s->d_enc, mats.data(), sizeof(sgrl_gemm::EncMat) * mats.size(), hipMemcpyHostToDevice) != hipSuccess)
      return sfail(SGRL_ERR_HIP, "device allocation failed in sgrl_set_bind_params (row-scale table)");
  }
  s->n_chunks = (int)chunks.size();
  s->w = s->wflat;
  std::memcpy(s->off, offsets, sizeof(int64_t) * SGRL_SET_NW);
  for (int k = 0; k < SGRL_SET_NSITES; k++) s->site_ptr[k] = s->wflat + offsets[SGRL_SET_NW + k];
  {
    const int64_t ow = offsets[SGRL_SET_NW + SGRL_SET_NSITES], ob = offsets[SGRL_SET_NW + SGRL_SET_NSITES + 1];
    const bool have = room(ow) >= 32 * 256;
    s->l2mf_w = have ? s->wflat + ow : nullptr;
    s->l2mf_b = have ? s->wflat + ob : nullptr;
  }
  s->live = true;
  s->have_w = true;
  return SGRL_OK;
}

int sgrl_set_graph(sgrl_set* s, int n_morph, const int32_t* morph_L, const int32_t* morph_count, const int32_t* trav,
                   const float* rel) {
  if (!s || n_morph <= 0 || !morph_L || !morph_count || !trav || !rel) return sfail(SGRL_ERR_ARG, "sgrl_set_graph: bad argument");
  std::vector<int32_t> key_i;
  size_t ntrav = 0, nrel = 0;
  for (int k = 0; k < n_morph; k++) {
    if (morph_L[k] < 2 || morph_L[k] > 14) return sfail(SGRL_ERR_LIMIT, "limb count must be in [2, 14]");
    if (morph_count[k] < 0) return sfail(SGRL_ERR_ARG, "negative morph_count");
    ntrav += 3 * (size_t)morph_L[k];
    nrel += 3 * (size_t)morph_L[k] * morph_L[k];
  }
  key_i.push_back(n_morph);
  key_i.insert(key_i.end(), morph_L, morph_L + n_morph);
  key_i.insert(key_i.end(), morph_count, morph_count + n_morph);
  key_i.insert(key_i.end(), trav, trav + ntrav);
  for (GraphCfg* c : s->cfgs)
    if (c->key_i == key_i && c->key_f.size() == nrel && std::memcmp(c->key_f.data(), rel, sizeof(float) * nrel) == 0)
      return use_cfg(s, c);
  std::vector<int32_t> node_env, node_limb, node_mnode, env_off, env_L, env_relb, m_off, m_L, travT;
  int TM = 0, relb_off = 0, env = 0, node = 0, Lmax = 0;
  std::vector<int> m_node0;
  for (int k = 0; k < n_morph; k++) {
    m_node0.push_back(TM);
    m_off.push_back(relb_off);
    m_L.push_back(morph_L[k]);
    TM += morph_L[k];
    relb_off += 2 * morph_L[k] * morph_L[k];
    if (morph_L[k] > Lmax) Lmax = morph_L[k];
  }
  travT.assign(3 * (size_t)TM, 0);
  {
    size_t tp = 0;
    for (int k = 0; k < n_morph; k++) {
      const int L = morph_L[k];
      for (int q = 0; q < 3; q++)
        for (int i = 0; i < L; i++) {
          const int v = trav[tp + q * L + i];
          if (v < 0 || v >= 15) return sfail(SGRL_ERR_ARG, "traversal index out of range");
          travT[(size_t)q * TM + m_node0[k] + i] = v;
        }
      tp += 3 * (size_t)L;
    }
  }
  for (int k = 0; k < n_morph; k++) {
    for (int c = 0; c < morph_count[k]; c++) {
      env_off.push_back(node);
      env_L.push_back(morph_L[k]);
      env_relb.push_back(m_off[k]);
      for (int i = 0; i < morph_L[k]; i++) {
        node_env.push_back(env);
        node_limb.push_back(i);
        node_mnode.push_back(m_node0[k] + i);
        node++;
      }
      env++;
    }
  }
  if (node == 0) return sfail(SGRL_ERR_ARG, "no environments");
  if ((int)s->cfgs.size() >= SGRL_SET_GRAPH_CACHE) {
    size_t lru = 0;
    for (size_t i = 1; i < s->cfgs.size(); i++) if (s->cfgs[i]->last_use < s->cfgs[lru]->last_use) lru = i;
    s->cfgs[lru]->release();
    s->generation++;
    delete s->cfgs[lru];
    s->cfgs.erase(s->cfgs.begin() + lru);
  }
  GraphCfg* c = new GraphCfg();
  c->key_i = std::move(key_i);
  c->key_f.assign(rel, rel + nrel);
  c->n_env = env; c->N = node; c->n_morph = n_morph; c->TM = TM; c->Lmax = Lmax;
  pick_split(env_off, node, &c->split_env, &c->split_node);
  bool ok = upload(&c->d_node_env, node_env) == 0 && upload(&c->d_node_limb, node_limb) == 0 &&
            upload(&c->d_node_mnode, node_mnode) == 0 && upload(&c->d_trav, travT) == 0 &&
            upload(&c->d_env_off, env_off) == 0 && upload(&c->d_env_L, env_L) == 0 && upload(&c->d_env_relb, env_relb) == 0 &&
            upload(&c->d_m_off, m_off) == 0 && upload(&c->d_m_L, m_L) == 0 && upload(&c->d_rel, c->key_f) == 0;
  if (ok) ok = hipMalloc(&c->d_relb, sizeof(float) * relb_off) == hipSuccess;
  if (!ok) { c->release(); delete c; return sfail(SGRL_ERR_HIP, "device allocation failed in sgrl_set_graph"); }
  s->cfgs.push_back(c);
  return use_cfg(s, c);
}

int sgrl_set_forward(sgrl_set* s, const float* obs, int obs_ld, float* act, int act_ld, float max_action, void* stream) {
  if (!s || !obs || !act) return sfail(SGRL_ERR_ARG, "sgrl_set_forward: null argument");
  if (!s->have_w || !s->have_graph) return sfail(SGRL_ERR_ARG, "sgrl_set_forward: weights or graph not set");
  if (obs_ld < 41 * s->Lmax || act_ld < 3 * s->Lmax)
    return sfail(SGRL_ERR_ARG, "sgrl_set_forward: obs_ld < 41 * Lmax or act_ld < 3 * Lmax (rows too narrow for the largest morphology)");
  return run_forward(s, obs, obs_ld, act, act_ld, max_action, (hipStream_t)stream);
}

int sgrl_set_forward_q(sgrl_set* s, const float* obs, int obs_ld, const float* action, int action_ld, float* q, int q_ld,
                       void* stream) {
  if (!s || !obs || !action || !q) return sfail(SGRL_ERR_ARG, "sgrl_set_forward_q: null argument");
  if (!s->have_w || !s->have_graph) return sfail(SGRL_ERR_ARG, "sgrl_set_forward_q: weights or graph not set");
  if (obs_ld < 41 * s->Lmax || action_ld < 3 * s->Lmax || q_ld < s->Lmax)
    return sfail(SGRL_ERR_ARG, "sgrl_set_forward_q: obs_ld < 41 * Lmax, action_ld < 3 * Lmax or q_ld < Lmax");
  return run_forward(s, obs, obs_ld, q, q_ld, 0.f, (hipStream_t)stream, true, action, action_ld);
}

int sgrl_set_time_forward(sgrl_set* s, const float* obs, int obs_ld, float* act, int act_ld, float max_action,
                          int reps, void* stream, float* ms_out) {
  if (!s || !obs || !act || !ms_out || reps <= 0) return sfail(SGRL_ERR_ARG, "sgrl_set_time_forward: bad argument");
  if (!s->have_w || !s->have_graph) return sfail(SGRL_ERR_ARG, "weights or graph not set");
  if (obs_ld < 41 * s->Lmax || act_ld < 3 * s->Lmax) return sfail(SGRL_ERR_ARG, "sgrl_set_time_forward: rows too narrow for the largest morphology");
  hipEvent_t t0, t1;
  SHIP_TRY(hipEventCreate(&t0));
  SHIP_TRY(hipEventCreate(&t1));
  SHIP_TRY(hipEventRecord(t0, (hipStream_t)stream));
  for (int r = 0; r < reps; r++) {
    int rc = run_forward(s, obs, obs_ld, act, act_ld, max_action, (hipStream_t)stream);
    if (rc != SGRL_OK) return rc;
  }
  SHIP_TRY(hipEventRecord(t1, (hipStream_t)stream));
  SHIP_TRY(hipEventSynchronize(t1));
  float ms = 0;
  SHIP_TRY(hipEventElapsedTime(&ms, t0, t1));
  (void)hipEventDestroy(t0);
  (void)hipEventDestroy(t1);
  *ms_out = ms / reps;
  return SGRL_OK;
}

int sgrl_set_hold_weights(sgrl_set* s, int hold) {
  if (!s) return sfail(SGRL_ERR_ARG, "sgrl_set_hold_weights: null handle");
  s->hold = hold != 0;
  s->packed_ok = false;
  return SGRL_OK;
}

int sgrl_set_num_nodes(const sgrl_set* s) { return s ? s->N : SGRL_ERR_ARG; }
int64_t sgrl_set_workspace_bytes(const sgrl_set* s) { return s ? s->ws_floats * 4 : -1; }
int64_t sgrl_set_generation(const sgrl_set* s) { return s ? s->generation : -1; }
int sgrl_set_last_split(const sgrl_set* s) { return s ? s->last_split : SGRL_ERR_ARG; }

int sgrl_set_peek(sgrl_set* s, int which, float* host, int64_t n_floats) {
  if (!s || !host || !s->have_graph) return sfail(SGRL_ERR_ARG, "sgrl_set_peek: bad argument");
  const float* src[] = {s->g, s->cat_cur ? s->cat_cur : s->cat, s->zc, s->fn, s->qkv, nullptr, nullptr, s->mat, s->g1, s->delta, s->outng};
  const int64_t per[] = {384, 256, 96, 1, 768, 0, 0, 96, 384, 128, 160};
  if (which < 0 || which > 10 || !src[which] || n_floats > per[which] * s->N) return sfail(SGRL_ERR_ARG, "sgrl_set_peek: bad buffer or size");
  SHIP_TRY(hipDeviceSynchronize());
  SHIP_TRY(hipMemcpy(host, src[which], sizeof(float) * n_floats, hipMemcpyDeviceToHost));
  return SGRL_OK;
}

int sgrl_set_debug_stop_after(sgrl_set* s, int stage) {
  if (!s || stage < -1 || stage >= 2 * SGRL_SET_LAYERS) return sfail(SGRL_ERR_ARG, "sgrl_set_debug_stop_after: bad argument");
  s->stop_after = stage;
  return SGRL_OK;
}

int sgrl_set_debug_small_nodes(sgrl_set* s, int nodes) {
  if (!s || nodes < -1) return sfail(SGRL_ERR_ARG, "sgrl_set_debug_small_nodes: bad argument");
  s->small_nodes = nodes;
  return SGRL_OK;
}

int sgrl_set_gemm_form(sgrl_set* s, int form) {
  if (!s || (form != 0 && form != SGRL_SET_FORM_F16X3 && form != SGRL_SET_FORM_BF16X6)) return sfail(SGRL_ERR_ARG, "sgrl_set_gemm_form: bad argument");
  if (s->gemm_form != form) s->generation++;
  s->gemm_form = form;
  return SGRL_OK;
}

namespace {
struct TempWords {
  unsigned* w = nullptr; float* sc = nullptr; sgrl_gemm::EncMat* dm = nullptr;
  ~TempWords() { if (w) (void)hipFree(w); if (sc) (void)hipFree(sc); if (dm) (void)hipFree(dm); }
  int make(hipStream_t st, const float* W, int rows, int K, int group = 1) {
    const sgrl_gemm::EncMat m{0, rows, K, 0, group};
    if (hipMalloc(&w, sizeof(unsigned) * (size_t)rows * K) != hipSuccess || hipMalloc(&sc, sizeof(float) * rows) != hipSuccess ||
        hipMalloc(&dm, sizeof(m)) != hipSuccess || hipMemcpy(dm, &m, sizeof(m), hipMemcpyHostToDevice) != hipSuccess)
      return sfail(SGRL_ERR_HIP, "debug product: allocation failed");
    hipLaunchKernelGGL(sgrl_gemm::k_encode_rows, dim3((rows + 3) / 4), dim3(256), 0, st, W, w, sc, dm, 1, rows);
    return SGRL_OK;
  }
};
}

int sgrl_set_debug_product(sgrl_set* s, int kind, int form, const float* A, int lda, const float* W, int ldw, const float* bias,
                           float* C, int ldc, int M, int N, int K, const float* rowdiv, const float* aux_in, float* aux_out,
                           void* stream) {
  if (!s || !A || !W || !C || M <= 0 || N <= 0 || K <= 0) return sfail(SGRL_ERR_ARG, "sgrl_set_debug_product: bad argument");
  hipStream_t st = (hipStream_t)stream;
  if (!GemmKernels<0>::raise_lds_limits() || !GemmKernels<EPI_RELU>::raise_lds_limits() || !GemmKernels<EPI_ROWDIV>::raise_lds_limits())
    return sfail(SGRL_ERR_HIP, "cannot raise the dynamic LDS limit of the tile kernels");
  TempWords tw;
  const std::vector<std::pair<int64_t, int>> index{{0, 0}};
  GemmCtx gx;
  gx.form = form == 1 ? SGRL_SET_FORM_BF16X6 : form;
  gx.w_base = W;
  if (form == SGRL_SET_FORM_F16X3) {
    if (ldw != K) return sfail(SGRL_ERR_ARG, "debug product: the two-piece form takes W rows of K contiguous floats");
    if (tw.make(st, W, N, K, kind == 4 ? 32 : 1) != SGRL_OK) return SGRL_ERR_HIP;
    gx.w_words = tw.w; gx.wsc = tw.sc; gx.enc_index = &index;
  }
  int rc = SGRL_OK;
  if (form == 1) {
    if (kind > 2 || (K % 16) != 0) rc = sfail(SGRL_ERR_ARG, "debug product: the exact-f32 kernel serves kinds 0..2");
    else {
      GemmArgs a{A, lda, W, ldw, bias, C, ldc, M, N, K, kind == 1 ? EPI_RELU : (kind == 2 ? EPI_ROWDIV : 0), rowdiv, nullptr, 0};
      const dim3 grid(((M + 127) / 128) * ((N + 63) / 64));
      if (kind == 0) hipLaunchKernelGGL(GemmKernels<0>::kNarrow, grid, dim3(256), GemmKernels<0>::kNarrowLds, st, a);
      else if (kind == 1) hipLaunchKernelGGL(GemmKernels<EPI_RELU>::kNarrow, grid, dim3(256), GemmKernels<0>::kNarrowLds, st, a);
      else hipLaunchKernelGGL(GemmKernels<EPI_ROWDIV>::kNarrow, grid, dim3(256), GemmKernels<0>::kNarrowLds, st, a);
    }
  } else if (kind <= 2) {
    if (N <= 64 || (K % 32) != 0) rc = sfail(SGRL_ERR_ARG, "debug product: the split kernels serve N > 64, K % 32 == 0");
    else rc = launch_gemm(gx, st, A, lda, W, ldw, bias, C, ldc, M, N, K, kind == 1 ? EPI_RELU : (kind == 2 ? EPI_ROWDIV : 0), rowdiv);
  } else if (kind == 3) {
    if (K != GK || ldw != GK || !aux_out) rc = sfail(SGRL_ERR_ARG, "debug product: Gram operand needs K = ldw = 576 and aux_out");
    else rc = launch_gemm_gram(gx, st, A, W, bias, C, ldc, M, N, aux_out);
  } else if (kind == 4) {
    if (N != 1024 || !rowdiv || !aux_in) rc = sfail(SGRL_ERR_ARG, "debug product: equivariant epilogue needs N = 1024, rowdiv, zq");
    else rc = launch_gemm_equiv(gx, st, A, lda, W, ldw, bias, M, K, rowdiv, aux_in, C);
  } else if (kind == 5) {
    if (N != 64 || !aux_out || (K % 16) != 0) rc = sfail(SGRL_ERR_ARG, "debug product: stacked projections need N = 64 and aux_out");
    else {
      GemmArgs a{A, lda, W, ldw, nullptr, C, ZD, M, 64, K, EPI_ZSPLIT, nullptr, aux_out, ZD};
      if (form == SGRL_SET_FORM_F16X3) {
        if (hipFuncSetAttribute(reinterpret_cast<const void*>(kProjH), hipFuncAttributeMaxDynamicSharedMemorySize, kProjHLds) != hipSuccess)
          rc = sfail(SGRL_ERR_HIP, "debug product: LDS limit");
        else hipLaunchKernelGGL(kProjH, dim3(((M + 127) / 128) * 1), dim3(256), kProjHLds, st, with_words(gx, a));
      } else if (GemmKernels<EPI_ZSPLIT>::raise_lds_limits()) GemmKernels<EPI_ZSPLIT>::launch(gx, st, a);
      else rc = sfail(SGRL_ERR_HIP, "debug product: LDS limit");
    }
  } else if (kind == 6) {
    if (N != 128 || !rowdiv || !aux_in) rc = sfail(SGRL_ERR_ARG, "debug product: LayerNorm epilogue needs N = 128, rowdiv, ln_w | ln_b");
    else rc = launch_gemm_ln(gx, st, A, lda, W, ldw, bias, M, K, rowdiv, C, ldc, aux_in, aux_in + 128);
  } else rc = sfail(SGRL_ERR_ARG, "debug product: unknown kind");
  const hipError_t le = hipGetLastError();
  if (rc == SGRL_OK && le != hipSuccess) rc = sfail(SGRL_ERR_HIP, std::string("debug product: launch failed: ") + hipGetErrorString(le));
  (void)hipStreamSynchronize(st);
  return rc;
}

int sgrl_set_debug_chain(sgrl_set* s, int kind, const float* A, int lda, int K, const float* Wp, const float* W1, const float* b1, int hid,
                         const float* W2, const float* b2, float* C, int ldc, int M, const float* rowdiv, const float* ln, float* zc,
                         float* z2, float* fn, void* stream) {
  if (!s || !A || !W1 || !W2 || !C || M <= 0 || K <= 0 || (K % 16) || (lda & 3) || (hid != 128 && hid != 256))
    return sfail(SGRL_ERR_ARG, "sgrl_set_debug_chain: bad argument");
  hipStream_t st = (hipStream_t)stream;
  if (!chain_raise_lds_limits()) return sfail(SGRL_ERR_HIP, "cannot raise the dynamic LDS limit of the chain kernels");
  TempWords t1, t2, tp;
  const int K1 = kind == 2 ? GK : K;
  if (t1.make(st, W1, hid, K1) != SGRL_OK || t2.make(st, W2, kind == 3 ? 1024 : 128, hid, kind == 3 ? 32 : 1) != SGRL_OK) return SGRL_ERR_HIP;
  ChainArgs a{};
  a.W1 = t1.w; a.ldw1 = K1; a.b1 = b1; a.W2 = t2.w; a.ldw2 = hid; a.b2 = b2; a.M = M; a.K1 = K1; a.ws1 = t1.sc; a.ws2 = t2.sc;
  const dim3 grid((M + sgrl_gemm::kChainRows - 1) / sgrl_gemm::kChainRows);
  int rc = SGRL_OK;
  if (kind == 0) {
    a.A = A; a.lda = lda; a.C = C; a.ldc = ldc;
    if (hid == 256) hipLaunchKernelGGL(kChainPlain, grid, dim3(512), sgrl_gemm::kChainLds, st, a);
    else hipLaunchKernelGGL(kChainNg, grid, dim3(512), sgrl_gemm::kChainLds, st, a);
  } else if (kind == 1) {
    if (hid != 256 || !rowdiv || !ln) rc = sfail(SGRL_ERR_ARG, "debug chain: the LayerNorm pair needs hid = 256, rowdiv, ln_w | ln_b");
    else {
      a.A = A; a.lda = lda; a.rowdiv = rowdiv; a.ln_io = C; a.ln_ld = ldc; a.ln_w = ln; a.ln_b = ln + 128;
      hipLaunchKernelGGL(kChainLn, grid, dim3(512), sgrl_gemm::kChainLds, st, a);
    }
  } else if (kind == 2) {
    if (!Wp || !zc || !fn) rc = sfail(SGRL_ERR_ARG, "debug chain: the site needs Wp, zc, fn");
    else if (tp.make(st, Wp, 64, K) != SGRL_OK) rc = SGRL_ERR_HIP;
    else {
      a.A = zc; a.C = C; a.ldc = ldc; a.fn_out = fn; a.X = A; a.ldx = lda; a.Kp = K; a.Wp = tp.w; a.wsp = tp.sc; a.zc = zc; a.z2 = z2;
      if (hid == 256) {
        if (z2) hipLaunchKernelGGL(kSiteF, grid, dim3(512), sgrl_gemm::kChainLds, st, a);
        else hipLaunchKernelGGL(kSiteA, grid, dim3(512), sgrl_gemm::kChainLds, st, a);
      } else {
        if (z2) hipLaunchKernelGGL(kSiteH2, grid, dim3(512), sgrl_gemm::kChainLds, st, a);
        else hipLaunchKernelGGL(kSiteH1, grid, dim3(512), sgrl_gemm::kChainLds, st, a);
      }
    }
  } else if (kind == 3) {
    if (hid != 256 || !rowdiv || !ln) rc = sfail(SGRL_ERR_ARG, "debug chain: the equivariant pair needs hid = 256, rowdiv, zq (in `ln`)");
    else {
      a.A = A; a.lda = lda; a.rowdiv = rowdiv; a.zq = ln; a.tout = C;
      hipLaunchKernelGGL(kChainEq, grid, dim3(512), sgrl_gemm::kChainEqLds, st, a);
    }
  } else rc = sfail(SGRL_ERR_ARG, "debug chain: unknown kind");
  const hipError_t le = hipGetLastError();
  if (rc == SGRL_OK && le != hipSuccess) rc = sfail(SGRL_ERR_HIP, std::string("debug chain: launch failed: ") + hipGetErrorString(le));
  (void)hipStreamSynchronize(st);
  return rc;
}

long long sgrl_set_debug_redos(int reset) {
  unsigned n = 0;
  if (hipDeviceSynchronize() != hipSuccess || hipMemcpyFromSymbol(&n, HIP_SYMBOL(sgrl_gemm::g_scale_redos), sizeof(n)) != hipSuccess) return -1;
  const unsigned zero = 0;
  if (reset && hipMemcpyToSymbol(HIP_SYMBOL(sgrl_gemm::g_scale_redos), &zero, sizeof(zero)) != hipSuccess) return -1;
  return (long long)n;
}

const char* sgrl_set_last_error(void) { return g_set_err.c_str(); }

}
```

### sgrl_amd/set_hip.py

```python
import ctypes

import numpy as np
import torch

from . import _lib

NGLOBAL, NLAYER, LAYERS = 25, 31, 3
NW = NGLOBAL + LAYERS * NLAYER


def _bind(L):
    if getattr(L, "_set_bound", False):
        return
    vp = ctypes.c_void_p
    L.sgrl_set_create.argtypes = [ctypes.POINTER(vp)]
    L.sgrl_set_destroy.argtypes = [vp]
    L.sgrl_set_destroy.restype = None
    L.sgrl_set_weights.argtypes = [vp, vp, vp, ctypes.c_int]
    L.sgrl_set_bind_params.argtypes = [vp, vp, ctypes.c_int, vp, ctypes.c_int, ctypes.c_int64]
    L.sgrl_set_graph.argtypes = [vp, ctypes.c_int, vp, vp, vp, vp]
    L.sgrl_set_forward.argtypes = [vp, vp, ctypes.c_int, vp, ctypes.c_int, ctypes.c_float, vp]
    L.sgrl_set_forward_q.argtypes = [vp, vp, ctypes.c_int, vp, ctypes.c_int, vp, ctypes.c_int, vp]
    L.sgrl_set_time_forward.argtypes = [vp, vp, ctypes.c_int, vp, ctypes.c_int, ctypes.c_float, ctypes.c_int, vp,
                                        ctypes.POINTER(ctypes.c_float)]
    L.sgrl_set_num_nodes.argtypes = [vp]
    L.sgrl_set_workspace_bytes.argtypes = [vp]
    L.sgrl_set_workspace_bytes.restype = ctypes.c_int64
    L.sgrl_set_generation.argtypes = [vp]
    L.sgrl_set_generation.restype = ctypes.c_int64
    L.sgrl_set_peek.argtypes = [vp, ctypes.c_int, vp, ctypes.c_int64]
    L.sgrl_set_debug_stop_after.argtypes = [vp, ctypes.c_int]
    L.sgrl_set_debug_small_nodes.argtypes = [vp, ctypes.c_int]
    L.sgrl_set_last_split.argtypes = [vp]
    L.sgrl_set_gemm_form.argtypes = [vp, ctypes.c_int]
    L.sgrl_set_last_error.restype = ctypes.c_char_p
    L.sgrl_set_hold_weights.argtypes = [vp, ctypes.c_int]
    L.sgrl_set_debug_redos.argtypes = [ctypes.c_int]
    L.sgrl_set_debug_redos.restype = ctypes.c_longlong
    ci = ctypes.c_int
    L.sgrl_set_debug_product.argtypes = [vp, ci, ci, vp, ci, vp, ci, vp, vp, ci, ci, ci, ci, vp, vp, vp, vp]
    L.sgrl_set_debug_chain.argtypes = [vp, ci, vp, ci, ci, vp, vp, vp, ci, vp, vp, vp, ci, ci, vp, vp, vp, vp, vp, vp]
    L._set_bound = True


def _check(L, rc, what):
    if rc != 0:
        raise _lib.SgrlError("%s failed (%d): %s" % (what, rc, L.sgrl_set_last_error().decode()))


GRAM_K = 576


def gram_order():
    a, b, ok = [], [], []
    for A in range(8):
        for B in range(A + 1):
            for i in range(4):
                for j in range(4):
                    a.append(4 * A + i); b.append(4 * B + j); ok.append(4 * A + i >= 4 * B + j)
    return torch.tensor(a), torch.tensor(b), torch.tensor(ok)


def fold_gram_weight(w):
    out_f = w.shape[0]
    w3 = w.reshape(out_f, 32, 32)
    sym = w3 + w3.transpose(1, 2)
    idx_a, idx_b, ok = gram_order()
    f = sym[:, idx_a, idx_b].clone()
    diag = idx_a == idx_b
    f[:, diag] = w3[:, idx_a[diag], idx_b[diag]]
    f[:, ~ok] = 0
    return f.contiguous()


def perm32(t):
    return t.reshape(32, 32, *t.shape[1:]).transpose(0, 1).reshape(t.shape).contiguous()


def pack_tensors(sd, prefix="actor.", critic=False):
    g = lambda k: sd[prefix + k].detach().float()
    out = [None] * NW
    out[0:3] = [g("pos_encoder.embeddings.%d.weight" % i) for i in range(3)]
    out[3], out[4] = g("transformer_encoder.rel_encoder.weight"), g("transformer_encoder.rel_encoder.bias")
    out[5], out[6] = g("transformer_encoder.norm.weight"), g("transformer_encoder.norm.bias")
    out[7], out[8], out[9] = g("g_encoder.weight"), g("encoder.weight"), g("encoder.bias")
    out[10] = g("gg_proj.weight")
    out[11], out[12], out[13], out[14] = fold_gram_weight(g("linear1_g.weight")), g("linear1_g.bias"), g("linear2_g.weight"), g("linear2_g.bias")
    w = g("linear1_ng.weight")
    out[15] = torch.cat([w, w.new_zeros(w.shape[0], 160 - w.shape[1])], dim=1)
    out[16], out[17], out[18] = g("linear1_ng.bias"), g("linear2_ng.weight"), g("linear2_ng.bias")
    if critic:
        z = w.new_zeros(1)
        out[19], out[21] = g("decoder_ng.weight").reshape(-1), g("decoder_ng.bias").reshape(-1)
        out[20], out[22], out[23], out[24] = z, z, z, z
    else:
        out[19] = g("decoder_g.weight").reshape(-1)
        out[20], out[21], out[22], out[23] = g("linear1_m.weight"), g("linear1_m.bias"), perm32(g("linear2_m.weight")), perm32(g("linear2_m.bias"))
        out[24] = g("g_proj.weight")
    scaling = float(128) ** -0.5
    for l in range(LAYERS):
        p = "transformer_encoder.layers.%d." % l
        a = p + "self_attn."
        b = NGLOBAL + l * NLAYER
        vg, wgo, wng = g(a + "vg_proj.weight"), g(a + "g_out.weight"), g(a + "ng_out.weight")
        wv, bv = g(a + "v_proj.weight"), g(a + "v_proj.bias")
        vfold = torch.cat([wng[:, 128 * h:128 * h + 128] @ wv[128 * h:128 * h + 128] for h in range(2)], 0)
        bfold = torch.cat([wng[:, 128 * h:128 * h + 128] @ bv[128 * h:128 * h + 128] for h in range(2)], 0)
        ufold = torch.cat([wgo[:, 128 * h:128 * h + 126] @ vg[126 * h:126 * h + 126] for h in range(2)], 0)
        gdcol = torch.stack([wgo[:, 128 * h + 126:128 * h + 128] for h in range(2)], 0).contiguous()
        out[b:b + NLAYER] = [
            g(a + "g_proj.weight"), fold_gram_weight(g(a + "linear_g1.weight")), g(a + "linear_g1.bias"), g(a + "linear_g2.weight"),
            g(a + "linear_g2.bias"),
            torch.cat([g(a + "q_proj.weight") * scaling, g(a + "k_proj.weight"), vfold], 0),
            torch.cat([g(a + "q_proj.bias") * scaling, g(a + "k_proj.bias"), bfold], 0),
            ufold,
            wng, g(a + "ng_out.bias"), wgo,
            g(p + "g_proj2.weight"), g(p + "g_proj3.weight"), fold_gram_weight(g(p + "linear_g1.weight")), g(p + "linear_g1.bias"),
            g(p + "linear_g2.weight"), g(p + "linear_g2.bias"), g(p + "linear3.weight"), g(p + "linear3.bias"),
            perm32(g(p + "linear4.weight")), perm32(g(p + "linear4.bias")), g(p + "linear5.weight"), g(p + "linear1.weight"),
            g(p + "linear1.bias"), g(p + "linear2.weight"), g(p + "linear2.bias"), g(p + "norm1.weight"),
            g(p + "norm1.bias"), g(p + "norm2.weight"), g(p + "norm2.bias"), gdcol]
    return out


NSITES = 7
NEXTRA = 2
PACK_COPY, PACK_PADCOL, PACK_FOLD, PACK_STACK, PACK_MATMUL, PACK_SUBMAT, PACK_PERM32 = 0, 1, 2, 3, 4, 5, 6
SEG_DTYPE = np.dtype([("dst", "<i8"), ("src0", "<u8"), ("src1", "<u8"), ("n", "<i4"), ("kind", "<i4"), ("a", "<i4"),
                      ("b", "<i4"), ("scale", "<f4"), ("lda", "<i4"), ("ldb", "<i4"), ("reserved", "<i4")])
assert SEG_DTYPE.itemsize == 56


def plan_segments(net, critic=False):
    sd = dict(net.named_parameters())
    segs, srcs, offs, pos = [], [], np.zeros(NW + NSITES + NEXTRA, dtype=np.int64), [0]

    def p(name):
        t = sd[name]
        assert t.dtype == torch.float32 and t.is_contiguous(), "SET parameters must be contiguous float32: " + name
        return t

    def emit(kind, t0, n, a=0, b=0, scale=1.0, t1=None, off0=0, off1=0, lda=0, ldb=0):
        segs.append((pos[0], t0.data_ptr() + 4 * off0, 0 if t1 is None else t1.data_ptr() + 4 * off1, n, kind, a, b, scale,
                     lda, ldb, 0))
        srcs.append((t0, t1, off0, off1))
        pos[0] += n

    anchor = p("g_encoder.weight")

    def align():
        fill = (-pos[0]) % 64
        if fill:
            emit(PACK_COPY, anchor, fill, a=0)

    def copy(name, scale=1.0, n=None):
        t = p(name)
        emit(PACK_COPY, t, t.numel() if n is None else n, a=t.numel(), scale=scale)

    def fold(name):
        t = p(name)
        assert t.shape[1] == 1024
        emit(PACK_FOLD, t, t.shape[0] * GRAM_K)

    def padcol(name, cols):
        t = p(name)
        emit(PACK_PADCOL, t, t.shape[0] * cols, a=t.shape[1], b=cols)

    def zero():
        emit(PACK_COPY, anchor, 64, a=0)

    def perm32(name):
        t = p(name)
        assert t.shape[0] == 1024
        emit(PACK_PERM32, t, t.numel(), a=t.numel() // 1024)

    def slot(i, fn, *args, **kw):
        align()
        offs[i] = pos[0]
        fn(*args, **kw)

    for i in range(3):
        slot(i, copy, "pos_encoder.embeddings.%d.weight" % i)
    slot(3, copy, "transformer_encoder.rel_encoder.weight"); slot(4, copy, "transformer_encoder.rel_encoder.bias")
    slot(5, copy, "transformer_encoder.norm.weight"); slot(6, copy, "transformer_encoder.norm.bias")
    slot(7, copy, "g_encoder.weight"); slot(8, copy, "encoder.weight"); slot(9, copy, "encoder.bias")
    slot(10, copy, "gg_proj.weight")
    slot(11, fold, "linear1_g.weight"); slot(12, copy, "linear1_g.bias")
    slot(13, copy, "linear2_g.weight"); slot(14, copy, "linear2_g.bias")
    slot(15, padcol, "linear1_ng.weight", 160); slot(16, copy, "linear1_ng.bias")
    slot(17, copy, "linear2_ng.weight"); slot(18, copy, "linear2_ng.bias")
    if critic:
        slot(19, copy, "decoder_ng.weight"); slot(20, zero); slot(21, copy, "decoder_ng.bias")
        slot(22, zero); slot(23, zero); slot(24, zero)
    else:
        slot(19, copy, "decoder_g.weight")
        slot(20, copy, "linear1_m.weight"); slot(21, copy, "linear1_m.bias")
        slot(22, perm32, "linear2_m.weight"); slot(23, perm32, "linear2_m.bias")
        slot(24, copy, "g_proj.weight")
    scaling = float(128) ** -0.5
    for l in range(LAYERS):
        lp = "transformer_encoder.layers.%d." % l
        at = lp + "self_attn."
        b0 = NGLOBAL + l * NLAYER

        wng, wgo = p(at + "ng_out.weight"), p(at + "g_out.weight")

        def qkv(kind):
            copy(at + "q_proj." + kind, scale=scaling); copy(at + "k_proj." + kind)
            v = p(at + "v_proj." + kind)
            for h in range(2):
                if kind == "weight":
                    emit(PACK_MATMUL, wng, 128 * 256, a=128, b=256, t1=v, off0=128 * h, off1=128 * h * 256, lda=256, ldb=256)
                else:
                    emit(PACK_MATMUL, wng, 128, a=128, b=1, t1=v, off0=128 * h, off1=128 * h, lda=256, ldb=1)

        def ufold():
            vgw = p(at + "vg_proj.weight")
            for h in range(2):
                emit(PACK_MATMUL, wgo, 128 * 128, a=126, b=128, t1=vgw, off0=128 * h, off1=126 * h * 128, lda=256, ldb=128)

        def gdcols():
            for h in range(2):
                emit(PACK_SUBMAT, wgo, 128 * 2, b=2, off0=128 * h + 126, lda=256)
        slot(b0 + 0, copy, at + "g_proj.weight")
        slot(b0 + 1, fold, at + "linear_g1.weight"); slot(b0 + 2, copy, at + "linear_g1.bias")
        slot(b0 + 3, copy, at + "linear_g2.weight"); slot(b0 + 4, copy, at + "linear_g2.bias")
        slot(b0 + 5, qkv, "weight"); slot(b0 + 6, qkv, "bias")
        slot(b0 + 7, ufold)
        slot(b0 + 8, copy, at + "ng_out.weight"); slot(b0 + 9, copy, at + "ng_out.bias")
        slot(b0 + 10, copy, at + "g_out.weight")
        slot(b0 + 11, copy, lp + "g_proj2.weight"); slot(b0 + 12, copy, lp + "g_proj3.weight")
        slot(b0 + 13, fold, lp + "linear_g1.weight"); slot(b0 + 14, copy, lp + "linear_g1.bias")
        slot(b0 + 15, copy, lp + "linear_g2.weight"); slot(b0 + 16, copy, lp + "linear_g2.bias")
        slot(b0 + 17, copy, lp + "linear3.weight"); slot(b0 + 18, copy, lp + "linear3.bias")
        slot(b0 + 19, perm32, lp + "linear4.weight"); slot(b0 + 20, perm32, lp + "linear4.bias")
        slot(b0 + 21, copy, lp + "linear5.weight")
        slot(b0 + 22, copy, lp + "linear1.weight"); slot(b0 + 23, copy, lp + "linear1.bias")
        slot(b0 + 24, copy, lp + "linear2.weight"); slot(b0 + 25, copy, lp + "linear2.bias")
        slot(b0 + 26, copy, lp + "norm1.weight"); slot(b0 + 27, copy, lp + "norm1.bias")
        slot(b0 + 28, copy, lp + "norm2.weight"); slot(b0 + 29, copy, lp + "norm2.bias")
        slot(b0 + 30, gdcols)

    def stack(w0, w1, cols, cpad):
        t0 = p(w0)
        assert tuple(t0.shape) == (30, cols)
        emit(PACK_STACK, t0, 64 * cpad, a=cols, b=cpad, t1=None if w1 is None else p(w1))

    for l in range(LAYERS):
        lp = "transformer_encoder.layers.%d." % l
        slot(NW + 2 * l, stack, lp + "self_attn.g_proj.weight", None, 128, 128)
        slot(NW + 2 * l + 1, stack, lp + "g_proj2.weight", lp + "g_proj3.weight", 128, 128)
    slot(NW + 6, stack, "gg_proj.weight", None if critic else "g_proj.weight", 136, 144)

    def head_fold(kind):
        wd, t = p("decoder_g.weight"), p("linear2_m." + kind)
        for q in range(32):
            if kind == "weight":
                emit(PACK_MATMUL, wd, 256, a=32, b=256, t1=t, off1=q * 32 * 256, lda=32, ldb=256)
            else:
                emit(PACK_MATMUL, wd, 1, a=32, b=1, t1=t, off1=q * 32, lda=32, ldb=1)
    if critic:
        slot(NW + 7, zero); slot(NW + 8, zero)
    else:
        slot(NW + 7, head_fold, "weight"); slot(NW + 8, head_fold, "bias")
    align()
    return np.array(segs, dtype=SEG_DTYPE), offs, pos[0], srcs


def graph_key(graph):
    return tuple(int(v) for v in graph["parents"])


class HipSetActor(object):

    def __init__(self, policy, device=None, net=None, critic=False):
        if not torch.cuda.is_available():
            raise _lib.SgrlError("HipSetActor needs an MI355X (no CPU fallback)")
        self.L = _lib.lib()
        _bind(self.L)
        self.policy = policy
        self.net = net if net is not None else policy.actor
        self.critic = bool(critic)
        self.device = torch.device(device) if device is not None else next(self.net.parameters()).device
        if self.device.type != "cuda":
            raise _lib.SgrlError("the SEPolicy must live on the GPU for the HIP path")
        h = ctypes.c_void_p()
        _check(self.L, self.L.sgrl_set_create(ctypes.byref(h)), "sgrl_set_create")
        self.h = h
        self._bound = None
        self._cfg_key = None
        self._cfg_info = {}
        self.n_env = 0
        self.act_ld = 0

    def __del__(self):
        try:
            if getattr(self, "h", None):
                self.L.sgrl_set_destroy(self.h)
                self.h = None
        except Exception:
            pass

    def sync_weights(self, force=False):
        ptrs = tuple(p.data_ptr() for p in self.net.parameters())
        if not force and ptrs == self._bound:
            return
        segs, offs, total, srcs = plan_segments(self.net, critic=self.critic)
        if not all(src[0].is_cuda for src in srcs):
            raise _lib.SgrlError("the SET network must live on the GPU for the HIP path")
        _check(self.L, self.L.sgrl_set_bind_params(self.h, ctypes.c_void_p(segs.ctypes.data), len(segs),
                                                   ctypes.c_void_p(offs.ctypes.data), len(offs), ctypes.c_int64(total)),
               "sgrl_set_bind_params")
        self._bound = ptrs

    def configure(self, graphs, counts):
        key = (tuple(graph_key(g) for g in graphs), tuple(int(c) for c in counts))
        if key == self._cfg_key:
            return
        args = self._cfg_info.get(key)
        if args is None:
            Ls, trav, rel = [], [], []
            for g in graphs:
                t = [np.asarray(v.cpu() if torch.is_tensor(v) else v, dtype=np.int32) for v in g["traversals"]]
                Ls.append(len(t[0]))
                trav.append(np.concatenate(t))
                r = g["relation"]
                rel.append(np.asarray(r.detach().cpu() if torch.is_tensor(r) else r, dtype=np.float32).reshape(-1))
            args = (np.asarray(Ls, dtype=np.int32), np.asarray(counts, dtype=np.int32),
                    np.ascontiguousarray(np.concatenate(trav), dtype=np.int32),
                    np.ascontiguousarray(np.concatenate(rel), dtype=np.float32))
            if len(self._cfg_info) >= 128:
                self._cfg_info.clear()
            self._cfg_info[key] = args
        Ls, cnt, trav, rel = args
        vp = lambda a: ctypes.c_void_p(a.ctypes.data)
        _check(self.L, self.L.sgrl_set_graph(self.h, len(Ls), vp(Ls), vp(cnt), vp(trav), vp(rel)), "sgrl_set_graph")
        self._cfg_key = key
        self.n_env = int(cnt.sum())
        self.max_limbs = int(Ls.max())
        self.num_nodes = self.L.sgrl_set_num_nodes(self.h)

    def _stream(self):
        return ctypes.c_void_p(torch.cuda.current_stream(self.device).cuda_stream)

    @staticmethod
    def _ld(t):
        return int(t.stride(0)) if t.shape[0] > 1 else int(t.shape[1])

    def forward_batch(self, obs, out=None, act_ld=None):
        assert obs.is_cuda and obs.dtype == torch.float32 and obs.dim() == 2 and obs.stride(1) == 1
        assert obs.shape[0] == self.n_env
        assert obs.shape[1] >= 41 * self.max_limbs, "observation rows narrower than 41 * max_limbs"
        self.sync_weights()
        act_ld = act_ld or 3 * self.max_limbs
        assert act_ld >= 3 * self.max_limbs, "action rows narrower than 3 * max_limbs"
        if out is None:
            out = torch.empty((self.n_env, act_ld), dtype=torch.float32, device=self.device)
        assert out.is_contiguous() and out.shape == (self.n_env, act_ld)
        _check(self.L, self.L.sgrl_set_forward(self.h, ctypes.c_void_p(obs.data_ptr()), self._ld(obs),
                                               ctypes.c_void_p(out.data_ptr()), int(act_ld),
                                               ctypes.c_float(float(self.policy.max_action)), self._stream()),
               "sgrl_set_forward")
        return out

    def forward_q(self, obs, action, out=None, q_ld=None):
        assert self.critic, "forward_q needs a handle created with critic=True"
        for t in (obs, action):
            assert t.is_cuda and t.dtype == torch.float32 and t.dim() == 2 and t.stride(1) == 1 and t.shape[0] == self.n_env
        assert obs.shape[1] >= 41 * self.max_limbs and action.shape[1] >= 3 * self.max_limbs
        self.sync_weights()
        q_ld = q_ld or self.max_limbs
        assert q_ld >= self.max_limbs
        if out is None:
            out = torch.empty((self.n_env, q_ld), dtype=torch.float32, device=self.device)
        assert out.is_contiguous() and out.shape == (self.n_env, q_ld)
        _check(self.L, self.L.sgrl_set_forward_q(self.h, ctypes.c_void_p(obs.data_ptr()), self._ld(obs),
                                                 ctypes.c_void_p(action.data_ptr()), self._ld(action),
                                                 ctypes.c_void_p(out.data_ptr()), int(q_ld), self._stream()),
               "sgrl_set_forward_q")
        return out

    def time_forward(self, obs, out, reps):
        self.sync_weights()
        ms = ctypes.c_float(0)
        _check(self.L, self.L.sgrl_set_time_forward(self.h, ctypes.c_void_p(obs.data_ptr()), self._ld(obs),
                                                    ctypes.c_void_p(out.data_ptr()), self._ld(out),
                                                    ctypes.c_float(float(self.policy.max_action)), int(reps),
                                                    self._stream(), ctypes.byref(ms)), "sgrl_set_time_forward")
        return float(ms.value)

    def forward_single(self, state, graph):
        B = state.shape[0]
        self.configure([graph], [B])
        return self.forward_batch(state.contiguous().float(), act_ld=3 * len(graph["parents"]))

    def debug_stop_after(self, stage):
        _check(self.L, self.L.sgrl_set_debug_stop_after(self.h, int(stage)), "sgrl_set_debug_stop_after")

    def debug_small_nodes(self, nodes):
        _check(self.L, self.L.sgrl_set_debug_small_nodes(self.h, int(nodes)), "sgrl_set_debug_small_nodes")

    def last_split(self):
        return int(self.L.sgrl_set_last_split(self.h))

    FORM_F16X3, FORM_BF16X6 = 2, 3

    def gemm_form(self, form):
        _check(self.L, self.L.sgrl_set_gemm_form(self.h, int(form)), "sgrl_set_gemm_form")

    def hold_weights(self, hold=True):
        self.sync_weights()
        _check(self.L, self.L.sgrl_set_hold_weights(self.h, 1 if hold else 0), "sgrl_set_hold_weights")

    def scale_redos(self, reset=True):
        return int(self.L.sgrl_set_debug_redos(1 if reset else 0))

    def peek(self, which, per_node):
        out = np.zeros((self.num_nodes, per_node), dtype=np.float32)
        _check(self.L, self.L.sgrl_set_peek(self.h, which, ctypes.c_void_p(out.ctypes.data), out.size), "sgrl_set_peek")
        return out


class HipSetCritic(object):

    def __init__(self, critic_module, device=None):
        self.q1 = HipSetActor(critic_module, device=device, net=critic_module.critic1, critic=True)
        self.q2 = HipSetActor(critic_module, device=device, net=critic_module.critic2, critic=True)

    def configure(self, graphs, counts):
        self.q1.configure(graphs, counts)
        self.q2.configure(graphs, counts)

    def forward_batch(self, obs, action, q_ld=None, which=(1, 2)):
        out = []
        if 1 in which:
            out.append(self.q1.forward_q(obs, action, q_ld=q_ld))
        if 2 in which:
            out.append(self.q2.forward_q(obs, action, q_ld=q_ld))
        return tuple(out)

    def forward_single(self, state, action, graph, which=(1, 2)):
        B, L = state.shape[0], len(graph["parents"])
        self.configure([graph], [B])
        return self.forward_batch(state.contiguous().float(), action.contiguous().float(), q_ld=L, which=which)
```

Baseline: 1.930 million env-steps/s.

## Fold layer-0 geometric projections into precomputed weights and skip relbias when cached

Adds a device kernel that, after each weight pack, algebraically folds layer 0's g_proj, g_encoder, gram linear_g1 and vg_proj/g_out products into small precomputed matrices. The embed kernel then writes a compact 8-wide vector per node, the z-features and the norm directly. Layer-0 attention uses the folded 8-term update instead of the full vg GEMM, and the first site becomes a K=48 chain. This removes the layer-0 vg projection GEMM and shrinks the first MLP input. It also skips k_relbias when held weights and the graph are unchanged. The cost is added complexity, a double-precision fold kernel on every repack, and possible small numerical drift from the reassociated maths.

```diff
diff --git a/include/sgrl_set.h b/include/sgrl_set.h
--- a/include/sgrl_set.h
+++ b/include/sgrl_set.h
@@ -46,7 +46,7 @@
   int32_t reserved;
 } sgrl_pack_seg;
 #define SGRL_SET_NSITES 7
-#define SGRL_SET_NEXTRA 2
+#define SGRL_SET_NEXTRA 3
 int sgrl_set_bind_params(sgrl_set* s, const sgrl_pack_seg* segs, int n_segs, const int64_t* offsets, int n_offsets,
                          int64_t total_floats);
 
@@ -70,6 +70,7 @@
 int sgrl_set_debug_stop_after(sgrl_set* s, int stage);
 int sgrl_set_debug_small_nodes(sgrl_set* s, int nodes);
 int sgrl_set_last_split(const sgrl_set* s);
+int sgrl_set_debug_l0fold(sgrl_set* s, int on);
 #define SGRL_SET_FORM_F16X3 2
 #define SGRL_SET_FORM_BF16X6 3
 int sgrl_set_gemm_form(sgrl_set* s, int form);
diff --git a/sgrl_amd/csrc/set_actor.hip b/sgrl_amd/csrc/set_actor.hip
--- a/sgrl_amd/csrc/set_actor.hip
+++ b/sgrl_amd/csrc/set_actor.hip
@@ -53,11 +53,14 @@
   int TM;
 };
 constexpr int kEmbedNodes = 8;
+constexpr int kL0fW1 = 0, kL0fMt = 256 * 48, kL0fQ = kL0fMt + 8 * ZD, kL0fWu = kL0fQ + 64, kL0fFloats = kL0fWu + 128 * 2 * 8;
 __global__ __launch_bounds__(128) void k_embed(const float* __restrict__ obs, int obs_ld, const float* __restrict__ action,
                                                int act_ld, int ngf, NodeTab nt, const float* Wge, const float* We,
                                                const float* be, const float* e0, const float* e1, const float* e2, float* g,
-                                               float* cat, float* outg, float* outng, float* gdir, float* zc, float* z2, int N) {
+                                               float* cat, float* outg, float* outng, float* gdir, float* zc, float* z2, int N,
+                                               const float* __restrict__ l0f, float* vpad, float* fn) {
   __shared__ float os[kEmbedNodes][44];
+  __shared__ float sq[kEmbedNodes * 9];
   const int n0 = blockIdx.x * kEmbedNodes, c = threadIdx.x;
   for (int idx = c; idx < kEmbedNodes * 44; idx += 128) {
     const int q = idx / 44, k = idx % 44, n = n0 + q;
@@ -75,6 +78,8 @@
 #pragma unroll
   for (int j = 0; j < 20; j++) we[j] = j < ngf ? We[c * ngf + j] : 0.f;
   const float bias = be[c];
+  __shared__ float mq[8 * ZD + 64];
+  if (l0f) for (int k = c; k < 8 * ZD + 64; k += 128) mq[k] = l0f[kL0fMt + k];
   __syncthreads();
   const float sc = sqrtf(128.f);
   for (int q = 0; q < kEmbedNodes; q++) {
@@ -105,6 +110,41 @@
       gdir[((size_t)n * 3 + s) * 2 + e] = gv;
       zc[((size_t)n * 3 + s) * ZD + 30 + e] = gv;
       z2[((size_t)n * 3 + s) * ZD + 30 + e] = gv;
+    }
+  }
+  if (l0f) {
+    const int live = min(kEmbedNodes, N - n0) * 96;
+#pragma unroll 1
+    for (int idx = c; idx < live; idx += 128) {
+      const int q = idx / 96, s = (idx >> 5) % 3, col = idx & 31;
+      const float* o = os[q];
+      vpad[(size_t)n0 * 96 + idx] = col < 8 ? o[3 * col + s] : 0.f;
+      if (col < 30) {
+        float z = 0.f;
+#pragma unroll
+        for (int j = 0; j < 8; j++) z += o[3 * j + s] * mq[j * ZD + col];
+        zc[(size_t)n0 * 96 + idx] = z;
+      }
+    }
+    const float* Q = mq + 8 * ZD;
+    if (c < kEmbedNodes * 9) {
+      const float* o = os[c / 9];
+      const int s = (c % 9) / 3, s2 = c % 3;
+      float v = 0.f;
+#pragma unroll 1
+      for (int a = 0; a < 8; a++) {
+        float qa = 0.f;
+#pragma unroll
+        for (int b = 0; b < 8; b++) qa += Q[a * 8 + b] * o[3 * b + s2];
+        v += o[3 * a + s] * qa;
+      }
+      sq[c] = v * v;
+    }
+    __syncthreads();
+    if (c < kEmbedNodes && n0 + c < N) {
+      float ss = 0.f;
+      for (int k = 0; k < 9; k++) ss += sq[c * 9 + k];
+      fn[n0 + c] = sqrtf(ss) + 1.f;
     }
   }
 }
@@ -191,6 +231,71 @@
   }
 }
 
+constexpr int kFoldL0Blocks = 256 + 1 + 8;
+__global__ __launch_bounds__(256) void k_fold_l0(const float* __restrict__ Wp, const float* __restrict__ Wge, const float* __restrict__ W1,
+                                                 const float* __restrict__ Wu, const float* __restrict__ GD,
+                                                 const unsigned short* __restrict__ tri, float* out) {
+  __shared__ double mt[8][ZD];
+  __shared__ double tp[4][64];
+  const int t = threadIdx.x, blk = blockIdx.x;
+  const double sc = sqrt(128.0);
+  if (blk <= 256) {
+    const int a = t >> 5, x = t & 31;
+    double v = 0.0;
+    if (x < 30) {
+      double v4[4] = {0.0, 0.0, 0.0, 0.0};
+      for (int k = 0; k < D; k += 4)
+#pragma unroll
+        for (int u = 0; u < 4; u++) v4[u] += (double)Wp[x * D + k + u] * (double)Wge[(k + u) * 8 + a];
+      v = ((v4[0] + v4[1]) + (v4[2] + v4[3])) * sc;
+    } else {
+      v = (a == x - 29) ? 1.0 : 0.0;
+    }
+    mt[a][x] = v;
+    __syncthreads();
+  }
+  if (blk < 256) {
+    const int ab = t & 63, a = ab >> 3, b = ab & 7, part = t >> 6;
+    const float* row = W1 + (size_t)blk * GK;
+    double a4[4] = {0.0, 0.0, 0.0, 0.0};
+    for (int k = part * (GK / 4); k < (part + 1) * (GK / 4); k += 4)
+#pragma unroll
+      for (int u = 0; u < 4; u++) {
+        const unsigned tt = tri[k + u];
+        if (tt != 0xFFFFu) a4[u] += (double)row[k + u] * mt[a][tt >> 8] * mt[b][tt & 255];
+      }
+    tp[part][ab] = (a4[0] + a4[1]) + (a4[2] + a4[3]);
+    __syncthreads();
+    if (t < 48) {
+      const int kb = t >> 4, i = (t >> 2) & 3, j = t & 3;
+      const int ca = 4 * (kb > 0) + i, cb = 4 * (kb > 1) + j;
+      auto T = [&](int p, int q) { return (tp[0][p * 8 + q] + tp[1][p * 8 + q]) + (tp[2][p * 8 + q] + tp[3][p * 8 + q]); };
+      double v;
+      if (ca == cb) v = T(ca, ca);
+      else if (kb == 1) v = T(ca, cb) + T(cb, ca);
+      else v = 0.5 * (T(ca, cb) + T(cb, ca));
+      out[kL0fW1 + blk * 48 + t] = (float)v;
+    }
+  } else if (blk == 256) {
+    out[kL0fMt + t] = (float)mt[t >> 5][t & 31];
+    if (t < 64) {
+      double q = 0.0;
+      for (int x = 0; x < ZD; x++) q += mt[t >> 3][x] * mt[t & 7][x];
+      out[kL0fQ + t] = (float)q;
+    }
+  } else {
+    const int idx = (blk - 257) * 256 + t, c = idx & 127, p = (idx >> 7) & 7, h = idx >> 10;
+    const float* row = Wu + (size_t)(128 * h + c) * D;
+    double v4[4] = {0.0, 0.0, 0.0, 0.0};
+    for (int k = 0; k < D; k += 4)
+#pragma unroll
+      for (int u = 0; u < 4; u++) v4[u] += (double)row[k + u] * (double)Wge[(k + u) * 8 + p];
+    double v = ((v4[0] + v4[1]) + (v4[2] + v4[3])) * sc;
+    if (p == 1 || p == 2) v += (double)GD[(h * 128 + c) * 2 + (p - 1)];
+    out[kL0fWu + idx] = (float)v;
+  }
+}
+
 __global__ void k_relbias(const float* rel, const float* Wr, const float* br, float* relb, const int32_t* m_off,
                           const int32_t* m_L, int n_morph) {
   const int k = blockIdx.x;
@@ -208,6 +313,7 @@
   const int32_t* env_L;
   const int32_t* env_relb;
 };
+template <bool L0>
 __global__ __launch_bounds__(256) void k_attention(const float* __restrict__ qkv, const float* __restrict__ U,
                                                    const float* __restrict__ gdir, const float* relb, EnvTab et,
                                                    int use_bias, const float* __restrict__ b_ng, const float* __restrict__ GD,
@@ -215,7 +321,7 @@
                                                    const float* __restrict__ ln_w, const float* __restrict__ ln_b) {
   constexpr int LMAX = 14;
   __shared__ float sc[2 * LMAX * LMAX];
-  __shared__ float gd[2 * LMAX * 3 * 2];
+  __shared__ float gd[2 * LMAX * 3 * (L0 ? 8 : 2)];
   __shared__ float dl[LMAX][128];
   const int e = blockIdx.x, t = threadIdx.x;
   const int n0 = et.env_off[e], L = et.env_L[e];
@@ -245,25 +351,51 @@
     for (int j = 0; j < L; j++) row[j] = row[j] / sum;
   }
   __syncthreads();
-  for (int idx = t; idx < 2 * L * 6; idx += 256) {
-    const int h = idx / (L * 6), i = (idx / 6) % L, se = idx % 6;
-    const float* w = sc + (h * L + i) * L;
-    float s = 0.f;
-    for (int j = 0; j < L; j++) s += w[j] * gdir[(size_t)(n0 + j) * 6 + se];
-    gd[idx] = s;
+  if (L0) {
+    for (int idx = t; idx < 2 * L * 24; idx += 256) {
+      const int h = idx / (L * 24), i = (idx / 24) % L, sp = idx % 24;
+      const float* w = sc + (h * L + i) * L;
+      const float* vr = U + (size_t)n0 * 96 + (sp >> 3) * ZD + (sp & 7);
+      float s = 0.f;
+      for (int j = 0; j < L; j++) s += w[j] * vr[(size_t)j * 96];
+      gd[idx] = s;
+    }
+  } else {
+    for (int idx = t; idx < 2 * L * 6; idx += 256) {
+      const int h = idx / (L * 6), i = (idx / 6) % L, se = idx % 6;
+      const float* w = sc + (h * L + i) * L;
+      float s = 0.f;
+      for (int j = 0; j < L; j++) s += w[j] * gdir[(size_t)(n0 + j) * 6 + se];
+      gd[idx] = s;
+    }
   }
   __syncthreads();
   {
     const int quantity = t >> 6, ln = t & 63, h = ln >> 5, c4 = (ln & 31) * 4;
-    const float* vbase = quantity == 0 ? qkv + (size_t)n0 * 768 + 512 + h * 128 + c4
-                                       : U + ((size_t)n0 * 3 + (quantity - 1)) * 256 + h * 128 + c4;
+    const float* vbase = (quantity == 0 || L0) ? qkv + (size_t)n0 * 768 + 512 + h * 128 + c4
+                                               : U + ((size_t)n0 * 3 + (quantity - 1)) * 256 + h * 128 + c4;
     auto body = [&](auto ltc, const int i0) __attribute__((always_inline)) {
       constexpr int LT = decltype(ltc)::value;
       float4 out[LT];
 #pragma unroll
       for (int i = 0; i < LT; i++) out[i] = make_float4(0.f, 0.f, 0.f, 0.f);
       const float* wh = sc + h * L * L;
-      if (L <= 8) {
+      if (L0 && quantity != 0) {
+#pragma unroll 1
+        for (int pb = 0; pb < 8; pb += 2) {
+          float4 wu[2];
+#pragma unroll
+          for (int k = 0; k < 2; k++) wu[k] = *reinterpret_cast<const float4*>(GD + (h * 8 + pb + k) * 128 + c4);
+#pragma unroll
+          for (int k = 0; k < 2; k++)
+#pragma unroll
+            for (int i = 0; i < LT; i++)
+              if (i0 + i < L) {
+                const float mv = gd[((h * L + i0 + i) * 3 + (quantity - 1)) * 8 + pb + k];
+                out[i].x += wu[k].x * mv; out[i].y += wu[k].y * mv; out[i].z += wu[k].z * mv; out[i].w += wu[k].w * mv;
+              }
+        }
+      } else if (L <= 8) {
 #pragma unroll
         for (int jb = 0; jb < 8; jb += 4) {
           if (jb >= L) break;
@@ -295,7 +427,7 @@
           v = vn;
         }
       }
-      if (quantity != 0) {
+      if (quantity != 0 && !L0) {
         const float4 ga = *reinterpret_cast<const float4*>(GD + (h * 128 + c4) * 2);
         const float4 gb = *reinterpret_cast<const float4*>(GD + (h * 128 + c4) * 2 + 4);
 #pragma unroll
@@ -457,6 +589,7 @@
   int32_t *d_env_off = nullptr, *d_env_L = nullptr, *d_env_relb = nullptr, *d_m_off = nullptr, *d_m_L = nullptr;
   float *d_rel = nullptr, *d_relb = nullptr;
   uint64_t last_use = 0;
+  uint64_t relb_epoch = 0;
   void release() {
     void* ptrs[] = {d_node_env, d_node_limb, d_node_mnode, d_trav, d_env_off, d_env_L, d_env_relb, d_m_off, d_m_L, d_rel, d_relb};
     for (void* q : ptrs) if (q) (void)hipFree(q);
@@ -486,9 +619,14 @@
   const float* site_ptr[SGRL_SET_NSITES];
   bool hold = false, packed_ok = false;
   int packed_form = 0;
+  bool packed_l0f = false;
   hipEvent_t ev_pack = nullptr;
   const float* l2mf_w = nullptr;
   const float* l2mf_b = nullptr;
+  const float* l0f = nullptr;
+  bool l0fold_off = false;
+  uint64_t pack_epoch = 1;
+  GraphCfg* cur = nullptr;
   unsigned short* d_tri = nullptr;
   bool stack_dirty = true;
   bool stack_critic = false;
@@ -530,6 +668,7 @@
   if (s->ws) (void)hipFree(s->ws);
   s->ws = nullptr; s->ws_floats = 0; s->carved_N = 0;
   s->have_graph = false;
+  s->cur = nullptr;
 }
 
 template <class T>
@@ -577,6 +716,7 @@
   s->d_env_off = c->d_env_off; s->d_env_L = c->d_env_L; s->d_env_relb = c->d_env_relb; s->d_m_off = c->d_m_off; s->d_m_L = c->d_m_L;
   s->d_rel = c->d_rel; s->d_relb = c->d_relb;
   c->last_use = ++s->use_clock;
+  s->cur = c;
   s->have_graph = true;
   return SGRL_OK;
 }
@@ -702,6 +842,7 @@
 using sgrl_gemm::ChainArgs;
 using sgrl_gemm::k_chain;
 constexpr auto kSiteA = k_chain<1, 256, 0, 1>;
+constexpr auto kSiteA0 = k_chain<1, 256, 0, 0>;
 constexpr auto kSiteF = k_chain<1, 256, 0, 2>;
 constexpr auto kSiteH1 = k_chain<1, 128, 0, 1>;
 constexpr auto kSiteH2 = k_chain<1, 128, 0, 2>;
@@ -709,7 +850,7 @@
 constexpr auto kChainNg = k_chain<0, 128, 0, 0>;
 constexpr auto kChainPlain = k_chain<0, 256, 0, 0>;
 bool chain_raise_lds_limits() {
-  const void* ks[] = {reinterpret_cast<const void*>(kSiteA), reinterpret_cast<const void*>(kSiteF), reinterpret_cast<const void*>(kSiteH1),
+  const void* ks[] = {reinterpret_cast<const void*>(kSiteA0), reinterpret_cast<const void*>(kSiteA), reinterpret_cast<const void*>(kSiteF), reinterpret_cast<const void*>(kSiteH1),
                       reinterpret_cast<const void*>(kSiteH2), reinterpret_cast<const void*>(kChainLn), reinterpret_cast<const void*>(kChainNg),
                       reinterpret_cast<const void*>(kChainPlain)};
   for (const void* k : ks)
@@ -736,6 +877,15 @@
   }
   return SGRL_OK;
 }
+int launch_site0(const GemmCtx& gx, hipStream_t st, const float* V, const float* W1, const float* b1, const float* W2, const float* b2, float* C,
+                 int ldc, int M) {
+  ChainArgs a{};
+  a.A = V; a.W1 = words_of(gx, W1); a.ldw1 = 48; a.b1 = b1; a.W2 = words_of(gx, W2); a.ldw2 = 256; a.b2 = b2; a.C = C; a.ldc = ldc; a.M = M; a.K1 = 48;
+  a.ws1 = wsc_of(gx, W1); a.ws2 = wsc_of(gx, W2);
+  if (!a.ws1 || !a.ws2) return sfail(SGRL_ERR_ARG, "site 0: a weight operand is not a matrix of the row-scale table");
+  hipLaunchKernelGGL(kSiteA0, dim3((M + sgrl_gemm::kChainRows - 1) / sgrl_gemm::kChainRows), dim3(512), sgrl_gemm::kChainLds, st, a);
+  return SGRL_OK;
+}
 int launch_chain_ln(const GemmCtx& gx, hipStream_t st, const float* A, int lda, int K1, const float* W1, const float* b1, const float* W2, const float* b2,
                     const float* rowdiv, float* ln_io, int ln_ld, const float* ln_w, const float* ln_b, int M, float* ln_out = nullptr) {
   if (K1 % 16 != 0 || (lda & 3)) return sfail(SGRL_ERR_ARG, "chain: K must be a multiple of 16 and rows 16-byte aligned");
@@ -831,6 +981,7 @@
   bool critic; const float* action; int action_ld;
   hipStream_t st, sd;
   bool capturing, one_stream;
+  bool l0fold = false;
   bool small, chain;
   int ngf;
   GemmCtx gx;
@@ -895,27 +1046,38 @@
     const int N = s->N;
     (void)hipMemsetAsync(act, 0, sizeof(float) * (size_t)s->n_env * act_ld, st);
     const bool want_words = !small && gx.form == SGRL_SET_FORM_F16X3 && gemm_use_split();
-    const bool reuse = s->live && s->hold && s->packed_ok && (!want_words || s->packed_form == SGRL_SET_FORM_F16X3) && !capturing;
+    const bool reuse = s->live && s->hold && s->packed_ok && (!want_words || s->packed_form == SGRL_SET_FORM_F16X3) && (!l0fold || s->packed_l0f) &&
+                       !capturing;
     if (reuse) (void)hipStreamWaitEvent(st, s->ev_pack, 0);
     if (s->live && !reuse)
       hipLaunchKernelGGL(k_pack, dim3(s->n_chunks), dim3(256), 0, st, s->d_segs, s->d_chunks, s->d_tri, s->wflat);
+    if (s->live && !reuse && l0fold)
+      hipLaunchKernelGGL(k_fold_l0, dim3(kFoldL0Blocks), dim3(256), 0, st, s->site_ptr[0], s->W(SGRL_SET_GENC), s->WL(0, SGRL_SET_A_LG1_W),
+                         s->WL(0, SGRL_SET_VG_W), s->WL(0, SGRL_SET_A_GD), s->d_tri, s->wflat + (s->l0f - s->wflat));
     const bool encode = s->live && !reuse && want_words;
     if (encode) {
       fork(whole);
       hipLaunchKernelGGL(sgrl_gemm::k_encode_rows, dim3((s->enc_rows + 3) / 4), dim3(256), 0, sd, s->wflat, s->wwords, s->wsc, s->d_enc, s->n_enc,
                          s->enc_rows);
     }
-    hipLaunchKernelGGL(k_relbias, dim3(s->n_morph), dim3(256), 0, st, s->d_rel, s->W(SGRL_SET_REL_W), s->W(SGRL_SET_REL_B),
-                       s->d_relb, s->d_m_off, s->d_m_L, s->n_morph);
+    if (s->live && !reuse && !capturing) s->pack_epoch++;
+    const bool holding = s->live && s->hold && !capturing;
+    const bool relb_cur = reuse && s->cur && s->cur->relb_epoch == s->pack_epoch;
+    if (!relb_cur)
+      hipLaunchKernelGGL(k_relbias, dim3(s->n_morph), dim3(256), 0, st, s->d_rel, s->W(SGRL_SET_REL_W), s->W(SGRL_SET_REL_B),
+                         s->d_relb, s->d_m_off, s->d_m_L, s->n_morph);
+    if (s->cur) s->cur->relb_epoch = holding ? s->pack_epoch : 0;
     hipLaunchKernelGGL(k_embed, dim3((N + kEmbedNodes - 1) / kEmbedNodes), dim3(128), 0, st, obs, obs_ld, action, action_ld, ngf, nt,
                        s->W(SGRL_SET_GENC), s->W(SGRL_SET_ENC_W), s->W(SGRL_SET_ENC_B), s->W(SGRL_SET_EMB0), s->W(SGRL_SET_EMB1),
-                       s->W(SGRL_SET_EMB2), s->g, s->cat, s->outg, s->outng, s->gdir, s->zc, s->z2, N);
+                       s->W(SGRL_SET_EMB2), s->g, s->cat, s->outg, s->outng, s->gdir, s->zc, s->z2, N, l0fold ? s->l0f : (const float*)nullptr,
+                       s->mat, s->fn);
     if (encode) join(whole);
     if (s->live && !reuse && !capturing) {
       s->packed_ok = s->hold;
       s->packed_form = want_words ? SGRL_SET_FORM_F16X3 : SGRL_SET_FORM_BF16X6;
-      if (s->hold) (void)hipEventRecord(s->ev_pack, st);
-    }
+      s->packed_l0f = l0fold;
+    }
+    if (holding && (!reuse || !relb_cur)) (void)hipEventRecord(s->ev_pack, st);
     s->cat_cur = s->cat;
     if (!s->live && (s->stack_dirty || s->stack_critic != critic)) {
       s->stack_critic = critic;
@@ -929,6 +1091,12 @@
     }
   }
   int attn_site(const Part& p, int l) const {
+    if (l == 0 && l0fold) {
+      int rc = launch_site0(gx, p.st, p.mat, s->l0f + kL0fW1, s->WL(l, SGRL_SET_A_LG1_B), s->WL(l, SGRL_SET_A_LG2_W), s->WL(l, SGRL_SET_A_LG2_B), p.catc, 256, p.M);
+      if (rc != SGRL_OK) return rc;
+      if (p.ev_site0) (void)hipEventRecord(p.ev_site0, p.st);
+      return gemm(p.st, p.catc, 256, s->WL(l, SGRL_SET_QKV_W), 256, s->WL(l, SGRL_SET_QKV_B), p.qkv, 768, p.M, 768, 256, EPI_ROWDIV, p.fn);
+    }
     fork(p);
     int rc = gemm(p.sd, p.g, D, s->WL(l, SGRL_SET_VG_W), D, nullptr, p.vg, 256, 3 * p.M, 256, D);
     if (rc == SGRL_OK)
@@ -943,9 +1111,14 @@
   }
   int attention(const Part& p, int l) const {
     const EnvTab etp{et.env_off + p.e0, et.env_L + p.e0, et.env_relb + p.e0};
-    hipLaunchKernelGGL(k_attention, dim3(p.ne), dim3(256), 0, p.st, s->qkv, s->vg, s->gdir, s->d_relb, etp, l == 0 ? 1 : 0,
-                       s->WL(l, SGRL_SET_NGOUT_B), s->WL(l, SGRL_SET_A_GD), s->stop_after == 2 * l ? s->delta : (float*)nullptr,
-                       s->g1, p.catc - 256 * (size_t)p.r0 + 128, 256, s->WL(l, SGRL_SET_N1_W), s->WL(l, SGRL_SET_N1_B));
+    if (l == 0 && l0fold)
+      hipLaunchKernelGGL(k_attention<true>, dim3(p.ne), dim3(256), 0, p.st, s->qkv, s->mat, s->gdir, s->d_relb, etp, 1, s->WL(l, SGRL_SET_NGOUT_B),
+                         s->l0f + kL0fWu, s->stop_after == 2 * l ? s->delta : (float*)nullptr, s->g1, p.catc - 256 * (size_t)p.r0 + 128, 256,
+                         s->WL(l, SGRL_SET_N1_W), s->WL(l, SGRL_SET_N1_B));
+    else
+      hipLaunchKernelGGL(k_attention<false>, dim3(p.ne), dim3(256), 0, p.st, s->qkv, s->vg, s->gdir, s->d_relb, etp, l == 0 ? 1 : 0,
+                         s->WL(l, SGRL_SET_NGOUT_B), s->WL(l, SGRL_SET_A_GD), s->stop_after == 2 * l ? s->delta : (float*)nullptr,
+                         s->g1, p.catc - 256 * (size_t)p.r0 + 128, 256, s->WL(l, SGRL_SET_N1_W), s->WL(l, SGRL_SET_N1_B));
     return s->stop_after == 2 * l ? kStop : SGRL_OK;
   }
   int ffn_site(const Part& p, int l) const {
@@ -1059,6 +1232,7 @@
   f.et = EnvTab{s->d_env_off, s->d_env_L, s->d_env_relb};
   f.small = N <= (s->small_nodes >= 0 ? s->small_nodes : kSmallNodesDefault);
   f.chain = !f.small && chain_enabled() && gemm_use_split() && f.gx.form == SGRL_SET_FORM_F16X3;
+  f.l0fold = f.chain && s->live && s->l0f && !s->l0fold_off;
   hipStreamCaptureStatus cap = hipStreamCaptureStatusNone;
   (void)hipStreamIsCapturing(st, &cap);
   static const bool serial_env = [] { const char* e = getenv("SGRL_SET_ONE_STREAM"); return e && e[0] == '1'; }();
@@ -1190,7 +1364,7 @@
   std::memcpy(s->off, offsets, sizeof(int64_t) * SGRL_SET_NW);
   s->have_w = true;
   s->live = false;
-  s->l2mf_w = nullptr; s->l2mf_b = nullptr;
+  s->l2mf_w = nullptr; s->l2mf_b = nullptr; s->l0f = nullptr;
   s->stack_dirty = true;
   return SGRL_OK;
 }
@@ -1265,6 +1439,7 @@
       add(o[SGRL_SET_L1_W], 256, 256); add(o[SGRL_SET_L2_W], 128, 256); add(o[SGRL_SET_L5_W], 128, 32);
     }
     for (int k = 0; k < SGRL_SET_NSITES; k++) add(offsets[SGRL_SET_NW + k], 64, k == 6 ? OGLD : 128);
+    if (room(offsets[SGRL_SET_NW + SGRL_SET_NSITES + 2]) >= kL0fFloats) add(offsets[SGRL_SET_NW + SGRL_SET_NSITES + 2] + kL0fW1, 256, 48);
     if (s->d_enc) (void)hipFree(s->d_enc);
     if (s->wsc) (void)hipFree(s->wsc);
     s->d_enc = nullptr; s->wsc = nullptr;
@@ -1282,6 +1457,8 @@
     const bool have = room(ow) >= 32 * 256;
     s->l2mf_w = have ? s->wflat + ow : nullptr;
     s->l2mf_b = have ? s->wflat + ob : nullptr;
+    const int64_t of = offsets[SGRL_SET_NW + SGRL_SET_NSITES + 2];
+    s->l0f = room(of) >= kL0fFloats ? s->wflat + of : nullptr;
   }
   s->live = true;
   s->have_w = true;
@@ -1440,6 +1617,13 @@
 int sgrl_set_debug_small_nodes(sgrl_set* s, int nodes) {
   if (!s || nodes < -1) return sfail(SGRL_ERR_ARG, "sgrl_set_debug_small_nodes: bad argument");
   s->small_nodes = nodes;
+  return SGRL_OK;
+}
+
+int sgrl_set_debug_l0fold(sgrl_set* s, int on) {
+  if (!s) return sfail(SGRL_ERR_ARG, "sgrl_set_debug_l0fold: null handle");
+  if (s->l0fold_off != (on == 0)) s->generation++;
+  s->l0fold_off = on == 0;
   return SGRL_OK;
 }
 
diff --git a/sgrl_amd/set_hip.py b/sgrl_amd/set_hip.py
--- a/sgrl_amd/set_hip.py
+++ b/sgrl_amd/set_hip.py
@@ -33,6 +33,7 @@
     L.sgrl_set_debug_small_nodes.argtypes = [vp, ctypes.c_int]
     L.sgrl_set_last_split.argtypes = [vp]
     L.sgrl_set_gemm_form.argtypes = [vp, ctypes.c_int]
+    L.sgrl_set_debug_l0fold.argtypes = [vp, ctypes.c_int]
     L.sgrl_set_last_error.restype = ctypes.c_char_p
     L.sgrl_set_hold_weights.argtypes = [vp, ctypes.c_int]
     L.sgrl_set_debug_redos.argtypes = [ctypes.c_int]
@@ -124,7 +125,39 @@
 
 
 NSITES = 7
-NEXTRA = 2
+NEXTRA = 3
+L0F_W1, L0F_MT, L0F_Q, L0F_WU, L0F_FLOATS = 0, 256 * 48, 256 * 48 + 256, 256 * 48 + 320, 256 * 48 + 320 + 2048
+
+
+def layer0_fold(net):
+    sd = {k: v.detach().double().cpu().numpy() for k, v in net.named_parameters()}
+    at = "transformer_encoder.layers.0.self_attn."
+    wge, wp = sd["g_encoder.weight"], sd[at + "g_proj.weight"]
+    sc = np.sqrt(128.0)
+    mt = np.zeros((8, 32))
+    mt[:, :30] = sc * (wp @ wge).T
+    mt[1, 30] = mt[2, 31] = 1.0
+    w1 = fold_gram_weight(torch.from_numpy(sd[at + "linear_g1.weight"])).numpy()
+    ia, ib, ok = (t.numpy() for t in gram_order())
+    T = np.einsum("rk,ak,bk->rab", w1[:, ok], mt[:, ia[ok]], mt[:, ib[ok]])
+    S = T + T.transpose(0, 2, 1)
+    w1p = np.zeros((256, 48))
+    for blk, (A, B) in enumerate(((0, 0), (1, 0), (1, 1))):
+        for i in range(4):
+            for j in range(4):
+                a, b = 4 * A + i, 4 * B + j
+                w1p[:, 16 * blk + 4 * i + j] = T[:, a, a] if a == b else (S[:, a, b] if A != B else 0.5 * S[:, a, b])
+    wgo, wvg = sd[at + "g_out.weight"], sd[at + "vg_proj.weight"]
+    wu = np.zeros((128, 2, 8))
+    for h in range(2):
+        wu[:, h, :] = sc * (wgo[:, 128 * h:128 * h + 126] @ wvg[126 * h:126 * h + 126]) @ wge
+        wu[:, h, 1] += wgo[:, 128 * h + 126]
+        wu[:, h, 2] += wgo[:, 128 * h + 127]
+    return dict(Mt=mt, W1p=w1p, Q=mt @ mt.T, Wu=wu)
+
+
+def blocks48(C):
+    return np.concatenate([C[..., 4 * A:4 * A + 4, 4 * B:4 * B + 4].reshape(C.shape[:-2] + (16,)) for A, B in ((0, 0), (1, 0), (1, 1))], -1)
 PACK_COPY, PACK_PADCOL, PACK_FOLD, PACK_STACK, PACK_MATMUL, PACK_SUBMAT, PACK_PERM32 = 0, 1, 2, 3, 4, 5, 6
 SEG_DTYPE = np.dtype([("dst", "<i8"), ("src0", "<u8"), ("src1", "<u8"), ("n", "<i4"), ("kind", "<i4"), ("a", "<i4"),
                       ("b", "<i4"), ("scale", "<f4"), ("lda", "<i4"), ("ldb", "<i4"), ("reserved", "<i4")])
@@ -263,6 +296,7 @@
         slot(NW + 7, zero); slot(NW + 8, zero)
     else:
         slot(NW + 7, head_fold, "weight"); slot(NW + 8, head_fold, "bias")
+    slot(NW + 9, lambda: emit(PACK_COPY, anchor, L0F_FLOATS, a=0))
     align()
     return np.array(segs, dtype=SEG_DTYPE), offs, pos[0], srcs
 
@@ -400,6 +434,9 @@
     def debug_small_nodes(self, nodes):
         _check(self.L, self.L.sgrl_set_debug_small_nodes(self.h, int(nodes)), "sgrl_set_debug_small_nodes")
 
+    def debug_l0fold(self, on):
+        _check(self.L, self.L.sgrl_set_debug_l0fold(self.h, 1 if on else 0), "sgrl_set_debug_l0fold")
+
     def last_split(self):
         return int(self.L.sgrl_set_last_split(self.h))
 
```

Result: faster. 2.008 million env-steps/s, median of 6 (+4.1%).
